# opensensor/thingino-accel

Hardware: AMD Instinct MI355X
Metric: images/sec yolov5s_int8 640x640 batch256 (higher is better)
Workload: dtype int8

## Files before the change

### thingino-accel_amd/csrc/hip/conv_i8_common.hpp

```cpp
#pragma once
#include <hip/hip_runtime.h>
#include <stdint.h>
#include <stdlib.h>
#include <string.h>
#include <type_traits>

#include "../mhip.h"

extern "C" hipStream_t mhip_stream_native(void);
extern "C" int mhip_check(hipError_t e, const char *what);
extern "C" const void *mhip_zero_page(void);

typedef int v4i __attribute__((ext_vector_type(4)));
typedef int v2i __attribute__((ext_vector_type(2)));

#ifdef ANATOMY
struct anat_rec_t {
    unsigned key, wg, hwid, xcc;
    unsigned long long t[4];
};
static __device__ anat_rec_t *g_anat_buf;
static __device__ unsigned g_anat_cap;
#define ANAT_SETTER(NAME)                                                                                                    \
    extern "C" int NAME(void *buf, unsigned cap) {                                                                          \
// ... 82 lines not shown
    const uint32_t b = __builtin_amdgcn_perm((uint32_t)q3, (uint32_t)q2, 0x0c0c0400u);
    return (b << 16) | a;
}
__device__ __forceinline__ void lut4_at0(int q0, int q1, int q2, int q3, int &v0, int &v1, int &v2, int &v3) {
    asm volatile("ds_read_i8 %0, %4 offset:128\n\tds_read_i8 %1, %5 offset:128\n\t"
                 "ds_read_i8 %2, %6 offset:128\n\tds_read_i8 %3, %7 offset:128"
                 : "=&v"(v0), "=&v"(v1), "=&v"(v2), "=&v"(v3)
                 : "v"(q0), "v"(q1), "v"(q2), "v"(q3)
                 : "memory");
}
__device__ __forceinline__ void lds_base_must_be_zero(const void *dynamic_lds) {
    __builtin_amdgcn_s_setprio(3);
    unsigned a = (unsigned)(size_t)(const __attribute__((address_space(3))) void *)dynamic_lds;
    asm volatile("" : "+s"(a));
    if (a != 0u) __builtin_trap();
}
struct add_args_t {
    float s_conv, s_other, inv;
};
__device__ __forceinline__ int add_one(int v, uint32_t xword, int k, const add_args_t &g, int lo8, int hi8) {
    const int x = __builtin_amdgcn_sbfe((int)xword, 8 * k, 8);
    const float y = (float)v * g.s_conv + (float)x * g.s_other;
    const float t = y * g.inv;
    const int r = (int)(t + 0.5f);
    int m;
    asm("v_med3_i32 %0, %1, %2, %3" : "=v"(m) : "v"(r), "v"(lo8), "v"(hi8));
    return m;
}
__device__ __forceinline__ void lut4_fast(int q0, int q1, int q2, int q3, int &v0, int &v1, int &v2, int &v3) {
    asm volatile("ds_read_i8 %0, %4 offset:256\n\tds_read_i8 %1, %5 offset:256\n\t"
                 "ds_read_i8 %2, %6 offset:256\n\tds_read_i8 %3, %7 offset:256"
                 : "=&v"(v0), "=&v"(v1), "=&v"(v2), "=&v"(v3)
                 : "v"(q0), "v"(q1), "v"(q2), "v"(q3)
                 : "memory");
}
template <int NV>
__device__ __forceinline__ void requant_pack_pre(const int (&a)[NV], float cs, uint32_t (&pk)[NV / 4]) {
    const float cs2 = cs * 2.0f;
    const int klo = -256, khi = 255;
    int q[NV], v[NV];
#pragma unroll
    for (int i = 0; i < NV; i++) {
        const int k = (int)((float)a[i] * cs2);
        asm("v_med3_i32 %0, %1, %2, %3" : "=v"(q[i]) : "v"(k), "v"(klo), "v"(khi));
    }
#pragma unroll
    for (int g = 0; g < NV / 4; g++)
        asm volatile("ds_read_i8 %0, %4 offset:768\n\tds_read_i8 %1, %5 offset:768\n\t"
                     "ds_read_i8 %2, %6 offset:768\n\tds_read_i8 %3, %7 offset:768"
                     : "=&v"(v[4 * g]), "=&v"(v[4 * g + 1]), "=&v"(v[4 * g + 2]), "=&v"(v[4 * g + 3])
                     : "v"(q[4 * g]), "v"(q[4 * g + 1]), "v"(q[4 * g + 2]), "v"(q[4 * g + 3])
                     : "memory");
    wait_lds_values<NV>(v);
#pragma unroll
    for (int g = 0; g < NV / 4; g++) pk[g] = pack4(v[4 * g], v[4 * g + 1], v[4 * g + 2], v[4 * g + 3]);
}
__device__ __forceinline__ void requant_pack_two(const int (&a)[16], float cs0, float cs1, uint32_t (&pk)[4]) {
    const float c0 = cs0 * 2.0f, c1 = cs1 * 2.0f;
    const int klo = -256, khi = 255;
    int q[16], v[16];
#pragma unroll
    for (int i = 0; i < 16; i++) {
        const int k = (int)((float)a[i] * (i < 8 ? c0 : c1));
        asm("v_med3_i32 %0, %1, %2, %3" : "=v"(q[i]) : "v"(k), "v"(klo), "v"(khi));
    }
#pragma unroll
    for (int g = 0; g < 2; g++)
        asm volatile("ds_read_i8 %0, %4 offset:768\n\tds_read_i8 %1, %5 offset:768\n\t"
                     "ds_read_i8 %2, %6 offset:768\n\tds_read_i8 %3, %7 offset:768"
                     : "=&v"(v[4 * g]), "=&v"(v[4 * g + 1]), "=&v"(v[4 * g + 2]), "=&v"(v[4 * g + 3])
                     : "v"(q[4 * g]), "v"(q[4 * g + 1]), "v"(q[4 * g + 2]), "v"(q[4 * g + 3])
                     : "memory");
#pragma unroll
    for (int g = 2; g < 4; g++)
        asm volatile("ds_read_i8 %0, %4 offset:1280\n\tds_read_i8 %1, %5 offset:1280\n\t"
                     "ds_read_i8 %2, %6 offset:1280\n\tds_read_i8 %3, %7 offset:1280"
                     : "=&v"(v[4 * g]), "=&v"(v[4 * g + 1]), "=&v"(v[4 * g + 2]), "=&v"(v[4 * g + 3])
                     : "v"(q[4 * g]), "v"(q[4 * g + 1]), "v"(q[4 * g + 2]), "v"(q[4 * g + 3])
                     : "memory");
    wait_lds_values<16>(v);
#pragma unroll
    for (int g = 0; g < 4; g++) pk[g] = pack4(v[4 * g], v[4 * g + 1], v[4 * g + 2], v[4 * g + 3]);
}
template <int NV, bool HAS_LUT, bool SAFE, bool LUT0, bool ADD = false, bool FAST = false>
__device__ __forceinline__ void requant_pack(const int (&a)[NV], float cs, int lo, const uint8_t *lut128, uint32_t (&pk)[NV / 4],
                                             const uint32_t *xw = nullptr, const add_args_t *ga = nullptr) {
    int q[NV];
    const int hi = 127;
    if (FAST && HAS_LUT && LUT0 && SAFE) {
        const float cs2 = cs * 2.0f;
        const int klo = -256, khi = 255;
        int v[NV];
#pragma unroll
        for (int i = 0; i < NV; i++) {
            const int k = (int)((float)a[i] * cs2);
            asm("v_med3_i32 %0, %1, %2, %3" : "=v"(q[i]) : "v"(k), "v"(klo), "v"(khi));
        }
#pragma unroll
        for (int g = 0; g < NV / 4; g++)
            lut4_fast(q[4 * g], q[4 * g + 1], q[4 * g + 2], q[4 * g + 3], v[4 * g], v[4 * g + 1], v[4 * g + 2], v[4 * g + 3]);
        wait_lds_values<NV>(v);
        if (ADD) {
            const int lo8 = -128;
#pragma unroll
            for (int i = 0; i < NV; i++) v[i] = add_one(v[i], xw[i >> 2], i & 3, *ga, lo8, hi);
        }
#pragma unroll
        for (int g = 0; g < NV / 4; g++) pk[g] = pack4(v[4 * g], v[4 * g + 1], v[4 * g + 2], v[4 * g + 3]);
        return;
    }
#pragma unroll
    for (int i = 0; i < NV; i++) q[i] = SAFE ? requant_safe(a[i], cs, lo, hi) : requant<false>(a[i], cs, lo);
    if (HAS_LUT && LUT0) {
        int v[NV];
#pragma unroll
        for (int g = 0; g < NV / 4; g++)
            lut4_at0(q[4 * g], q[4 * g + 1], q[4 * g + 2], q[4 * g + 3], v[4 * g], v[4 * g + 1], v[4 * g + 2], v[4 * g + 3]);
        wait_lds_values<NV>(v);
        if (ADD) {
            const int lo8 = -128;
#pragma unroll
            for (int i = 0; i < NV; i++) v[i] = add_one(v[i], xw[i >> 2], i & 3, *ga, lo8, hi);
        }
#pragma unroll
        for (int g = 0; g < NV / 4; g++) pk[g] = pack4(v[4 * g], v[4 * g + 1], v[4 * g + 2], v[4 * g + 3]);
    } else {
        if (HAS_LUT) {
#pragma unroll
            for (int i = 0; i < NV; i++) q[i] = (int8_t)lut128[q[i]];
        }
        if (ADD) {
            const int lo8 = -128;
#pragma unroll
            for (int i = 0; i < NV; i++) q[i] = add_one(q[i], xw[i >> 2], i & 3, *ga, lo8, hi);
        }
#pragma unroll
        for (int g = 0; g < NV / 4; g++) pk[g] = pack4(q[4 * g], q[4 * g + 1], q[4 * g + 2], q[4 * g + 3]);
    }
}

struct fastdiv_t {
    unsigned m, s1, s2;
};
__device__ __forceinline__ unsigned fdiv(unsigned n, const fastdiv_t d) {
    const unsigned q = __umulhi(d.m, n);
    return (q + ((n - q) >> d.s1)) >> d.s2;
}
static fastdiv_t make_fastdiv(unsigned d) {
    fastdiv_t r;
    unsigned l = 0;
    while ((1ull << l) < d) l++;
    r.m = (unsigned)(((1ull << 32) * ((1ull << l) - d)) / d + 1);
    r.s1 = l < 1 ? l : 1;
    r.s2 = l > 0 ? l - 1 : 0;
    return r;
}

template <int N>
__device__ __forceinline__ void wait_vmcnt() {
    asm volatile("s_waitcnt vmcnt(%0)" ::"n"(N) : "memory");
}

__device__ __forceinline__ void glds16(const void *gsrc, void *lds_wave_base) {
    __builtin_amdgcn_global_load_lds((const __attribute__((address_space(1))) void *)gsrc,
                                     (__attribute__((address_space(3))) void *)lds_wave_base, 16, 0, 0);
}
// ... 187 lines not shown
```

### thingino-accel_amd/csrc/hip/conv_i8_patch.hip

```cpp
#include "conv_i8_common.hpp"
#include <stdio.h>

#ifdef PATCH_STAMPS
__device__ unsigned long long patch_stamp_sums[8];
extern "C" int mhip_patch_stamps(unsigned long long *out, int reset) {
    if (out && hipMemcpyFromSymbol(out, HIP_SYMBOL(patch_stamp_sums), sizeof(patch_stamp_sums)) != hipSuccess) return -1;
    if (reset) {
        unsigned long long z[8] = {0};
        if (hipMemcpyToSymbol(HIP_SYMBOL(patch_stamp_sums), z, sizeof(z)) != hipSuccess) return -1;
    }
    return 0;
}
#define STAMP(t)                                                                          \
    do {                                                                                  \
        __builtin_amdgcn_sched_barrier(0);                                                \
        asm volatile("s_memtime %0\n\ts_waitcnt lgkmcnt(0)" : "=s"(t)::"memory");        \
        __builtin_amdgcn_sched_barrier(0);                                                \
    } while (0)
#else
#define STAMP(t) do { } while (0)
#endif
#define PT_TW 16
#define PT_NIMAX 10

template <int LO, int HI>
__device__ __forceinline__ void wait_vmcnt_tree(int n) {
    if constexpr (LO == HI) {
        wait_vmcnt<LO>();
    } else {
        constexpr int MID = (LO + HI + 1) / 2;
        if (n >= MID) wait_vmcnt_tree<MID, HI>(n);
        else wait_vmcnt_tree<LO, MID - 1>(n);
    }
}
template <int HI>
__device__ __forceinline__ void wait_vmcnt_upto(int n) {
    wait_vmcnt_tree<0, HI>(n > HI ? HI : n);
}
__device__ __forceinline__ void barrier_lds() {
    asm volatile("s_waitcnt lgkmcnt(0)\n\ts_barrier" ::: "memory");
}

template <int TH, int BN, bool HAS_LUT, bool PRE = false, bool POST = false, bool SPLIT = false>
__global__ __launch_bounds__(NTHREADS) void conv_i8_patch(const mhip_conv_i8_t p, const int k64, const int tiles_x,
                                                          const int tiles_y, const unsigned ntiles_all, const int PH,
                                                          const int PW, const int PWP, const int PWH, const int nblk,
                                                          const int8_t *__restrict__ zeros, const fastdiv_t dtx,
                                                          const fastdiv_t dty, const fastdiv_t dpwp, const unsigned out_bytes,
                                                          const int ring, const int xmap, const unsigned in_bytes) {
    ANAT_BEGIN();
    constexpr int WPX = TH / 4;
    constexpr int WOC = BN / 16;
    constexpr int NST = WPX;
    extern __shared__ __attribute__((aligned(16))) int8_t dynlds[];
    uint8_t *slut = (uint8_t *)dynlds;
    lds_base_must_be_zero(dynlds);
    const int nks = k64 / BK;
    constexpr int NPO = 2 * BN;
    static_assert(!SPLIT || (BN == 64 && HAS_LUT && !PRE && !POST), "SPLIT: one 64-channel tile, no other stage");
    constexpr int LB = LUTB + ((PRE || POST) ? 512 : 0) + (SPLIT ? 1024 : 0);
    int *dutab = (int *)(dynlds + LB);
    int8_t *wl = dynlds + LB + ((nks * 16 + 255) & ~255);
    const int patch_bytes = nblk * 1024;
    int8_t *w1l = wl + nks * BN * BK;
    int8_t *pwl = w1l;
    const int *pbl = (const int *)(pwl + NPO * NPO);
    int8_t *swl = w1l;
    const int *sbl = (const int *)(swl + 64 * BK);
    int8_t *patch0 = w1l + (PRE ? p.in_c * BK : 0) + (POST ? NPO * NPO + NPO * 4 : 0) + (SPLIT ? 64 * BK + 64 * 4 : 0);
    int8_t *tpatch = patch0 + ring * patch_bytes;

    const int tid = threadIdx.x, lane = tid & 63;
    const int wv = __builtin_amdgcn_readfirstlane(tid >> 6);
    const int oc0 = blockIdx.y * BN;
    const int C = p.in_c, lgc = 31 - __builtin_clz((unsigned)C), cpp = C >> 4, lgcpp = lgc - 4;
    const int s = p.stride_w;
    const unsigned M = C >= 128 ? 6u : (C >= 64 ? 2u : 0u);

    v4i bias[WOC];
#pragma unroll
    for (int q = 0; q < WOC; q++) bias[q] = p.bias ? *(const v4i *)(p.bias + oc0 + q * 16 + (lane >> 4) * 4) : (v4i){0, 0, 0, 0};
    constexpr int W1MAX = 4;
    v4i pbias[PRE ? W1MAX : 1];
    if (PRE) {
#pragma unroll
        for (int q = 0; q < W1MAX; q++) pbias[q] = q < (C >> 4) ? *(const v4i *)(p.pre_bias + q * 16 + (lane >> 4) * 4) : (v4i){0, 0, 0, 0};
    }
    if (HAS_LUT) {
        if (p.lut2) { if (tid < 128) ((uint32_t *)slut)[tid] = ((const uint32_t *)p.lut2)[tid]; }
        else if (tid < 64) ((uint32_t *)slut)[tid] = ((const uint32_t *)p.lut)[tid];
    }
    if (PRE && tid >= 128) ((uint32_t *)slut)[tid] = ((const uint32_t *)p.pre_lut2)[tid - 128];
    if (POST) {
        if (tid >= 128) ((uint32_t *)slut)[tid] = ((const uint32_t *)p.post_lut2)[tid - 128];
        if (tid < NPO) ((int *)(pwl + NPO * NPO))[tid] = ((const int *)(p.post_w + NPO * NPO))[tid];
    }
    if (SPLIT) {
        if (tid >= 128) {
            ((uint32_t *)slut)[tid] = ((const uint32_t *)p.split_lut2[0])[tid - 128];
            ((uint32_t *)slut)[tid + 128] = ((const uint32_t *)p.split_lut2[1])[tid - 128];
        }
        if (tid < 64) ((int *)(swl + 64 * BK))[tid] = ((const int *)(p.split_w + 64 * BK))[tid];
    }
    const int rowbytes = p.kw * C, kbytes = p.kh * rowbytes;
    for (int i = tid; i < nks * 4; i += NTHREADS) {
        const int kb = i * 16;
        int du = 0;
        if (kb < kbytes) {
            const int ky = kb / rowbytes, rem = kb - ky * rowbytes, kx = rem >> lgc, cc = (rem & (C - 1)) >> 4;
            const int dp = ky * PWP + (s == 2 ? (kx >> 1) + (kx & 1) * PWH : kx);
            du = dp * cpp + cc;
        }
        dutab[i] = du;
    }
    __syncthreads();
    {
        const int schunk = (lane & 3) ^ (((lane >> 4) & 1) << 1);
        for (int i = wv; i < nks * (BN / 16); i += 4) {
            const int ks = i / (BN / 16), g = i - ks * (BN / 16);
            glds16(p.w + (size_t)(oc0 + g * 16 + (lane >> 2)) * k64 + ks * BK + schunk * 16, wl + (ks * BN + g * 16) * BK);
        }
        if (PRE)
            for (int g = wv; g < C / 16; g += 4) glds16(p.pre_w + (size_t)(g * 16 + (lane >> 2)) * BK + schunk * 16, w1l + g * 16 * BK);
        if (POST)
            for (int i = wv; i < NPO * NPO / 1024; i += 4) glds16(p.post_w + i * 1024 + lane * 16, pwl + i * 1024);
        if (SPLIT)
            glds16(p.split_w + wv * 1024 + lane * 16, swl + wv * 1024);
    }
    int uoff[PT_NIMAX], upos[PT_NIMAX];
#pragma unroll
    for (int n = 0; n < PT_NIMAX; n++) {
        uoff[n] = 0;
        upos[n] = -1;
        if (n * 4 + wv < nblk) {
            const unsigned phys = (unsigned)((n * 4 + wv) * 64 + lane);
            const unsigned U = phys ^ ((phys >> 3) & M);
            const unsigned pp = U >> lgcpp, cc = U & (unsigned)(cpp - 1);
            const unsigned py = fdiv(pp, dpwp), col = pp - py * (unsigned)PWP;
            const int px = s == 2 ? ((int)col < PWH ? 2 * (int)col : 2 * ((int)col - PWH) + 1) : (int)col;
            if ((int)py < PH && px < PW) {
                uoff[n] = ((int)py * p.in_w + px) * C + (int)cc * 16;
                upos[n] = ((int)py << 16) | px;
            }
        }
    }
    const int npw = nblk > wv ? (nblk - wv + 3) >> 2 : 0;
    const unsigned xcd = blockIdx.x & 7u;
    const unsigned xstart = xmap ? (unsigned)(((unsigned long long)ntiles_all * xcd) >> 3) : 0u;
    const unsigned xend = xmap ? (unsigned)(((unsigned long long)ntiles_all * (xcd + 1u)) >> 3) : 0u;
    const unsigned ntiles = xmap ? (xend - xstart) * 8u + xcd : ntiles_all;
    auto tile_xy = [&](unsigned t, int &tx, int &ty, unsigned &f) {
        const unsigned j = xmap ? xstart + (t >> 3) : t, q = fdiv(j, dtx);
        tx = (int)(j - q * (unsigned)tiles_x);
        f = fdiv(q, dty);
        ty = (int)(q - f * (unsigned)tiles_y);
    };
    const __amdgpu_buffer_rsrc_t xrs = __builtin_amdgcn_make_buffer_rsrc((void *)p.in, 0, (int)in_bytes, 0x00020000);
    auto issue_patch = [&](unsigned t, int8_t *dst) {
#ifdef PATCH_ABL
        return;
#endif
        int tx, ty;
        unsigned f;
        tile_xy(t, tx, ty, f);
        const int iy0 = ty * TH * s - p.pad_top, ix0 = tx * PT_TW * s - p.pad_left;
        if (in_bytes != 0u && iy0 >= 0 && ix0 >= 0 && iy0 + PH <= p.in_h && ix0 + PW <= p.in_w) {
            const int sbase = (int)(f * (unsigned)p.in_stride) + (iy0 * p.in_w + ix0) * C;
#pragma unroll
            for (int n = 0; n < PT_NIMAX; n++)
                if (n * 4 + wv < nblk) blds16(xrs, uoff[n], sbase, dst + (n * 4 + wv) * 1024);
            return;
        }
        const int8_t *base = p.in + (size_t)f * p.in_stride + ((long)iy0 * p.in_w + ix0) * C;
#pragma unroll
        for (int n = 0; n < PT_NIMAX; n++)
            if (n * 4 + wv < nblk) {
                const int py = upos[n] >> 16, px = upos[n] & 0xffff;
                const bool ok = upos[n] >= 0 && (unsigned)(iy0 + py) < (unsigned)p.in_h && (unsigned)(ix0 + px) < (unsigned)p.in_w;
                glds16(ok ? base + uoff[n] : zeros, dst + (n * 4 + wv) * 1024);
            }
    };

    const __amdgpu_buffer_rsrc_t orsrc = __builtin_amdgcn_make_buffer_rsrc(SPLIT ? p.split_out[0] : (POST ? p.post_out : p.out), 0, (int)out_bytes, 0x00020000);
    const unsigned out_bytes1 = SPLIT ? (unsigned)(p.frames - 1) * (unsigned)p.split_out_stride[1] + (unsigned)(p.out_h * p.out_w) * 32u : 0u;
    const __amdgpu_buffer_rsrc_t orsrc1 = __builtin_amdgcn_make_buffer_rsrc(SPLIT ? p.split_out[1] : p.out, 0, (int)out_bytes1, 0x00020000);
    const bool has_add = !SPLIT && p.add != nullptr;
    constexpr int RROW = WOC == 4 ? 1024 : 512;
    constexpr int NRI = WOC == 4 ? WPX : 2 * WPX;
    int8_t *rstage = patch0 + (ring + (PRE ? 1 : 0)) * patch_bytes + wv * (WPX * RROW);
    const int frow = lane & 15, fchunk = lane >> 4;
    const int chan = (lane >> 4) * (4 * WOC);
    const int NR = has_add || POST ? NRI : 0;
    const int ntail = POST ? (has_add ? NRI : 0) + WPX * (NPO / 64) : (SPLIT ? 2 * WPX : NST);
    const int ppstride = p.post_out_pix_stride ? p.post_out_pix_stride : NPO;
    auto issue_rows = [&](const int8_t *base, size_t fstride, int tx, int ty, unsigned f) {
#pragma unroll
        for (int u = 0; u < WPX; u++) {
            const int oy = ty * TH + wv * WPX + u, ox = tx * PT_TW + frow;
            const int8_t *src = oy < p.out_h && ox < p.out_w ? base + (size_t)f * fstride + ((size_t)(oy * p.out_w + ox) * BN + (size_t)chan) : zeros;
            if (WOC == 4) {
                glds16(src, rstage + u * RROW);
            } else {
                __builtin_amdgcn_global_load_lds((const __attribute__((address_space(1))) void *)src,
                                                 (__attribute__((address_space(3))) void *)(rstage + u * RROW), 4, 0, 0);
                __builtin_amdgcn_global_load_lds((const __attribute__((address_space(1))) void *)(src + 4),
                                                 (__attribute__((address_space(3))) void *)(rstage + u * RROW + 256), 4, 0, 0);
            }
        }
    };
    const int pstride = p.out_pix_stride ? p.out_pix_stride : p.out_c;
    const int lo = p.relu ? 0 : -128;
    const uint8_t *lut128 = slut + 128;
    int ubase[WPX];
#pragma unroll
    for (int u = 0; u < WPX; u++) ubase[u] = ((wv * WPX + u) * s * PWP + frow) * cpp;

    const unsigned G = gridDim.x;
    const int D = ring - 1;
    unsigned t = blockIdx.x;
    int yg0 = 0, yg1 = 0, yg2 = 0;
    {
        int issued = 0;
        for (int d = 0; d < D; d++)
            if (t + (unsigned)d * G < ntiles) {
                issue_patch(t + (unsigned)d * G, patch0 + d * patch_bytes);
                issued++;
            }
        yg0 = issued > 1 ? (issued - 1) * npw : 0;
        yg1 = issued > 2 ? (issued - 2) * npw : 0;
        yg2 = 0;
    }
#ifdef PATCH_STAMPS
    unsigned long long st0 = 0, st1 = 0, st2 = 0, st3 = 0, st4 = 0, sum_wait = 0, sum_issue = 0, sum_k = 0, sum_epi = 0, sum_tiles = 0;
#endif
    int cur = 0;
    int pn_last = 0;
    bool first = true;
    ANAT_NOW(1);
    for (; t < ntiles; t += G) {
        STAMP(st0);
        int tx, ty;
        unsigned f;
        tile_xy(t, tx, ty, f);
        int voffs[WPX];
        uint32_t xw[WPX][WOC];
#pragma unroll
        for (int u = 0; u < WPX; u++) {
            const int oy = ty * TH + wv * WPX + u, ox = tx * PT_TW + frow;
            const unsigned off = f * (unsigned)p.out_stride + (unsigned)(oy * p.out_w + ox) * (unsigned)pstride +
                                 (unsigned)(p.out_ch_off + oc0 + chan);
            const bool ok = oy < p.out_h && ox < p.out_w && oc0 + chan < p.out_c;
            voffs[u] = ok ? (int)off : -1;
#pragma unroll
            for (int q = 0; q < WOC; q++) xw[u][q] = 0;
        }
        if (POST) {
#pragma unroll
            for (int u = 0; u < WPX; u++) {
                const int oy = ty * TH + wv * WPX + u, ox = tx * PT_TW + frow;
                const unsigned off = f * (unsigned)p.post_out_stride + (unsigned)(oy * p.out_w + ox) * (unsigned)ppstride +
                                     (unsigned)(p.post_out_ch_off + (lane >> 4) * (NPO / 4));
                voffs[u] = oy < p.out_h && ox < p.out_w ? (int)off : -1;
            }
            if (has_add) issue_rows(p.add, p.out_stride, tx, ty, f);
            else issue_rows(p.post_in, p.post_in_stride, tx, ty, f);
        } else if (SPLIT) {
#pragma unroll
            for (int u = 0; u < WPX; u++) {
                const int oy = ty * TH + wv * WPX + u, ox = tx * PT_TW + frow;
                voffs[u] = oy < p.out_h && ox < p.out_w ? (oy * p.out_w + ox) * 32 + (lane >> 4) * 8 : -1;
            }
        } else if (has_add) {
#pragma unroll
            for (int u = 0; u < WPX; u++) {
                const int8_t *src = voffs[u] >= 0 ? p.add + (unsigned)voffs[u] : zeros;
                if (WOC == 4) {
// ... 116 lines not shown
            du_n = dutab[clampk(ks + 2) * 4 + fchunk];
            __builtin_amdgcn_sched_barrier(0);
            mfma_step(xb, wb);
            __builtin_amdgcn_sched_barrier(0);
            load_frags(clampk(ks + 2), du_n, xb, wb);
            du_n = dutab[clampk(ks + 3) * 4 + fchunk];
            __builtin_amdgcn_sched_barrier(0);
            mfma_step(xa, wa);
            __builtin_amdgcn_sched_barrier(0);
        }
        if (ks < nks) mfma_step(xb, wb);
        STAMP(st3);
        if (D > 0) cur = cur + 1 == ring ? 0 : cur + 1;
        if (has_add) {
            if (D > 0) wait_vmcnt_upto<15>(pn_last);
#pragma unroll
            for (int u = 0; u < WPX; u++) {
                if (WOC == 4) {
                    const v4i r = *(const v4i *)(rstage + u * RROW + lane * 16);
                    xw[u][0] = (uint32_t)r[0]; xw[u][1] = (uint32_t)r[1]; xw[u][WOC > 2 ? 2 : 0] = (uint32_t)r[2]; xw[u][WOC > 3 ? 3 : 0] = (uint32_t)r[3];
                } else {
                    xw[u][0] = *(const uint32_t *)(rstage + u * RROW + lane * 4);
                    xw[u][WOC > 1 ? 1 : 0] = *(const uint32_t *)(rstage + u * RROW + 256 + lane * 4);
                }
            }
        }
        uint32_t pku[POST || SPLIT ? WPX : 1][WOC];
        if (POST && has_add) {
#pragma unroll
            for (int u = 0; u < WPX; u++) {
                if constexpr (WOC == 4) asm volatile("s_waitcnt lgkmcnt(0)" : "+v"(xw[u][0]), "+v"(xw[u][1]), "+v"(xw[u][2]), "+v"(xw[u][3])::"memory");
                else asm volatile("s_waitcnt lgkmcnt(0)" : "+v"(xw[u][0]), "+v"(xw[u][1])::"memory");
            }
            issue_rows(p.post_in, p.post_in_stride, tx, ty, f);
        }
#pragma unroll
        for (int u = 0; u < WPX; u++) {
            uint32_t pk[WOC];
            int a[WOC * 4];
#pragma unroll
            for (int q = 0; q < WOC; q++)
#pragma unroll
                for (int r = 0; r < 4; r++) a[q * 4 + r] = acc[q][u][r];
            const bool fast = HAS_LUT && p.lut2 != nullptr;
            if (has_add) {
                const add_args_t ga = {p.add_s_conv, p.add_s_other, p.add_inv};
                if (fast) requant_pack<WOC * 4, HAS_LUT, true, true, true, true>(a, p.cs, lo, lut128, pk, xw[u], &ga);
                else requant_pack<WOC * 4, HAS_LUT, true, true, true>(a, p.cs, lo, lut128, pk, xw[u], &ga);
            } else {
                if (fast) requant_pack<WOC * 4, HAS_LUT, true, true, false, true>(a, p.cs, lo, lut128, pk);
                else requant_pack<WOC * 4, HAS_LUT, true, true>(a, p.cs, lo, lut128, pk);
            }
            if (POST) {
#pragma unroll
                for (int q = 0; q < WOC; q++) pku[POST ? u : 0][q] = pk[q];
                continue;
            }
            if (SPLIT) {
#pragma unroll
                for (int q = 0; q < WOC; q++) pku[SPLIT ? u : 0][q] = pk[q];
                continue;
            }
            const int voff = voffs[u];
            if (WOC == 4)
                __builtin_amdgcn_raw_buffer_store_b128((v4i){(int)pk[0], (int)pk[1], (int)pk[2], (int)pk[3]}, orsrc, voff, 0, 0);
            else if (WOC == 2)
                __builtin_amdgcn_raw_buffer_store_b64((v2i){(int)pk[0], (int)pk[WOC > 1 ? 1 : 0]}, orsrc, voff, 0, 0);
        }
        if (SPLIT) {
            v4i sw4[4], sb4[4];
#pragma unroll
            for (int r = 0; r < 4; r++) {
                sw4[r] = *(const v4i *)(swl + lds_off(r * 16 + frow, fchunk));
                sb4[r] = *(const v4i *)(sbl + r * 16 + fchunk * 4);
            }
            v4i sc[WPX][4];
#pragma unroll
            for (int u = 0; u < WPX; u++) {
                const v4i b0 = {(int)pku[SPLIT ? u : 0][0], (int)pku[SPLIT ? u : 0][1], (int)pku[SPLIT ? u : 0][WOC > 2 ? 2 : 0], (int)pku[SPLIT ? u : 0][WOC > 3 ? 3 : 0]};
#pragma unroll
                for (int r = 0; r < 4; r++) sc[u][r] = __builtin_amdgcn_mfma_i32_16x16x64_i8(sw4[r], b0, sb4[r], 0, 0, 0);
            }
            const unsigned fo0 = f * (unsigned)p.split_out_stride[0], fo1 = f * (unsigned)p.split_out_stride[1];
#pragma unroll
            for (int u = 0; u < WPX; u++) {
                int a2[16];
#pragma unroll
                for (int r = 0; r < 4; r++)
#pragma unroll
                    for (int e = 0; e < 4; e++) a2[r * 4 + e] = sc[u][r][e];
                uint32_t pk4[4];
                requant_pack_two(a2, p.split_cs[0], p.split_cs[1], pk4);
                const int voff0 = voffs[u] >= 0 ? voffs[u] + (int)fo0 : -1, voff1 = voffs[u] >= 0 ? voffs[u] + (int)fo1 : -1;
                __builtin_amdgcn_raw_buffer_store_b64((v2i){(int)pk4[0], (int)pk4[1]}, orsrc, voff0, 0, 0);
                __builtin_amdgcn_raw_buffer_store_b64((v2i){(int)pk4[2], (int)pk4[3]}, orsrc1, voff1, 0, 0);
            }
        }
        if (POST) {
            if (has_add) wait_vmcnt<0>();
            else if (D > 0) wait_vmcnt_upto<15>(pn_last);
#pragma unroll
            for (int u = 0; u < WPX; u++) {
                v4i b0, b1 = {0, 0, 0, 0};
                if (WOC == 4) {
                    b0 = (v4i){(int)pku[POST ? u : 0][0], (int)pku[POST ? u : 0][1], (int)pku[POST ? u : 0][WOC > 2 ? 2 : 0], (int)pku[POST ? u : 0][WOC > 3 ? 3 : 0]};
                    b1 = *(const v4i *)(rstage + u * RROW + lane * 16);
                } else {
                    b0 = (v4i){(int)pku[POST ? u : 0][0], (int)pku[POST ? u : 0][WOC > 1 ? 1 : 0], *(const int *)(rstage + u * RROW + lane * 4),
                               *(const int *)(rstage + u * RROW + 256 + lane * 4)};
                }
#pragma unroll
                for (int h = 0; h < NPO / 64; h++) {
                    int a[16];
#pragma unroll
                    for (int s4 = 0; s4 < 4; s4++) {
                        const int row = (h * 4 + s4) * 16;
                        v4i c = *(const v4i *)(pbl + row + fchunk * 4);
                        c = __builtin_amdgcn_mfma_i32_16x16x64_i8(*(const v4i *)(pwl + lds_off(row + frow, fchunk)), b0, c, 0, 0, 0);
                        if (WOC == 4) c = __builtin_amdgcn_mfma_i32_16x16x64_i8(*(const v4i *)(pwl + NPO * BK + lds_off(row + frow, fchunk)), b1, c, 0, 0, 0);
#pragma unroll
                        for (int e = 0; e < 4; e++) a[s4 * 4 + e] = c[e];
                    }
                    uint32_t pk4[4];
                    requant_pack_pre<16>(a, p.post_cs, pk4);
                    const int voff = voffs[u] >= 0 ? voffs[u] + h * 16 : -1;
                    __builtin_amdgcn_raw_buffer_store_b128((v4i){(int)pk4[0], (int)pk4[1], (int)pk4[2], (int)pk4[3]}, orsrc, voff, 0, 0);
                }
            }
        }
#ifdef PATCH_STAMPS
        STAMP(st4);
        if (D == 0) st1 = st2;
        sum_wait += st1 - st0; sum_issue += st2 - st1; sum_k += st3 - st2; sum_epi += st4 - st3; sum_tiles += 1;
#endif
    }
    ANAT_NOW(2);
    ANAT_END(p);
#ifdef PATCH_STAMPS
    if (lane == 0) {
        atomicAdd(&patch_stamp_sums[0], sum_wait); atomicAdd(&patch_stamp_sums[1], sum_issue); atomicAdd(&patch_stamp_sums[2], sum_k);
        atomicAdd(&patch_stamp_sums[3], sum_epi); atomicAdd(&patch_stamp_sums[4], sum_tiles);
    }
#endif
}

ANAT_SETTER(mhip_anatomy_set_patch)
struct patch_geom_t {
    int bn, tiles_x, tiles_y, PH, PW, PWP, PWH, nblk, nks, ring;
    size_t lds;
};
static inline const tune_t &tune() { return conv_i8_tune_state(); }
static size_t patch_lds_budget(int bn) {
    const int kb = tune().patch_lds_kb;
    if (kb >= 16 && kb <= 160 && kb != 80) return (size_t)kb * 1024;
    return (size_t)(bn == 32 ? 53 : 80) * 1024;
}
static bool patch_geom(const mhip_conv_i8_t *p, int th, patch_geom_t *g) {
    const bool direct = conv_i8_direct_rows(p);
    const int C = p->in_c, s = p->stride_w;
    static const bool no_c16 = getenv("MARS_HIP_PATCH_NO_C16") != nullptr;
    if (!direct || !p->safe || (C != 16 && C != 32 && C != 64 && C != 128) || (C == 16 && (no_c16 || p->pre_w)) || (s != 1 && s != 2) || p->stride_h != s ||
        p->kh > 7 || p->kw > 7 || p->kh * p->kw < 2 || p->row_pad != p->kw * C || persist_out_bytes(p) > 0x7fffffffL)
        return false;
    const int k64 = (p->kh * p->row_pad + BK - 1) / BK * BK;
    g->nks = k64 / BK;
    g->bn = p->oc_pad % 64 == 0 ? 64 : 32;
    g->tiles_x = (p->out_w + PT_TW - 1) / PT_TW;
    g->tiles_y = (p->out_h + th - 1) / th;
    if ((double)p->out_h * p->out_w < (C == 128 ? 0.80 : 0.85) * (double)g->tiles_x * PT_TW * g->tiles_y * th) return false;
    g->PH = (th - 1) * s + p->kh;
    g->PW = (PT_TW - 1) * s + p->kw;
    g->PWH = s == 2 ? (g->PW + 1) / 2 : 0;
    g->PWP = s == 2 ? 2 * g->PWH : g->PW;
    const long units = (long)g->PH * g->PWP * (C / 16);
    g->nblk = (int)((units + 63) / 64);
    if (g->nblk > 4 * PT_NIMAX) return false;
    const bool pre = p->pre_w != nullptr;
    if (pre && (s != 1 || (C != 32 && C != 64) || !p->pre_bias || !p->pre_lut2 || !p->lut2)) return false;
    const bool post = p->post_w != nullptr;
    if (post) {
        const long ppstride = p->post_out_pix_stride ? p->post_out_pix_stride : 2 * g->bn;
        if (pre || s != 1 || p->out_c != g->bn || p->oc_pad != g->bn || p->out_pix_stride || p->out_ch_off || !p->lut2 || !p->post_lut2 || !p->post_in ||
            !p->post_out || ((p->post_out_pix_stride | p->post_out_ch_off) & 15) || p->post_out_pix_stride < 0 || p->post_out_ch_off < 0 ||
            ppstride < p->post_out_ch_off + 2 * g->bn ||
            (long)(p->frames - 1) * (long)p->post_out_stride + (long)p->out_h * p->out_w * ppstride > 0x7fffffffL)
            return false;
    }
    const bool split = p->split_w != nullptr;
    if (split) {
        if (pre || post || p->add || g->bn != 64 || p->out_c != 64 || p->oc_pad != 64 || p->out_pix_stride || p->out_ch_off || !p->lut2 || !p->split_lut2[0] ||
            !p->split_lut2[1] || !p->split_out[0] || !p->split_out[1])
            return false;
        for (int i = 0; i < 2; i++)
            if ((long)(p->frames - 1) * (long)p->split_out_stride[i] + (long)p->out_h * p->out_w * 32 > 0x7fffffffL) return false;
    }
    const size_t pb = (size_t)g->nblk * 1024;
    const size_t radd = p->add || post ? (size_t)4 * (th / 4) * (g->bn == 64 ? 1024 : 512) : 0;
    const size_t fixed = LUTB + (pre ? 512 + (size_t)C * BK + pb : 0) + (post ? 512 + (size_t)4 * g->bn * g->bn + (size_t)8 * g->bn : 0) +
                         (split ? 1024 + (size_t)64 * BK + 64 * 4 : 0) +
                         (((size_t)g->nks * 16 + 255) & ~(size_t)255) + (size_t)g->nks * g->bn * BK + radd;
    const size_t budget = patch_lds_budget(g->bn);
    if (fixed + pb > budget) return false;
    const int fit = (int)((budget - fixed) / pb);
    const int cap = tune().patch_ring > 0 ? (tune().patch_ring > 4 ? 4 : tune().patch_ring) : 2;
    int ring = fit < cap ? fit : cap;
    g->ring = ring;
    g->lds = fixed + (size_t)ring * pb;
    if ((long)g->tiles_x * g->tiles_y * p->frames > 0x7fffffffL) return false;
    return true;
}

static inline long post_out_bytes(const mhip_conv_i8_t *p) {
    const long ppstride = p->post_out_pix_stride ? p->post_out_pix_stride : 2 * p->out_c;
    return (long)(p->frames - 1) * (long)p->post_out_stride + (long)p->out_h * p->out_w * ppstride;
}
static inline long split_out_bytes(const mhip_conv_i8_t *p, int side) {
    return (long)(p->frames - 1) * (long)p->split_out_stride[side] + (long)p->out_h * p->out_w * 32;
}
template <int TH, int BN, bool HAS_LUT, bool PRE = false, bool POST = false, bool SPLIT = false>
static int launch_patch_t(const mhip_conv_i8_t *p, int k64, const patch_geom_t &g) {
    auto kern = conv_i8_patch<TH, BN, HAS_LUT, PRE, POST, SPLIT>;
    static int cus = 0;
    static size_t slots_lds[8];
    static int slots_n[8], nslots = 0;
    if (!cus) {
        int dev = 0;
        hipDeviceProp_t prop;
        if (hipFuncSetAttribute((const void *)kern, hipFuncAttributeMaxDynamicSharedMemorySize, 160 * 1024) != hipSuccess ||
            hipGetDevice(&dev) != hipSuccess || hipGetDeviceProperties(&prop, dev) != hipSuccess)
            return mhip_check(hipErrorUnknown, "conv_i8_patch occupancy query");
        cus = prop.multiProcessorCount;
    }
    int slots = 0;
    for (int i = 0; i < nslots; i++)
        if (slots_lds[i] == g.lds) slots = slots_n[i];
    if (!slots) {
        int occ = 0;
        if (hipOccupancyMaxActiveBlocksPerMultiprocessor(&occ, kern, NTHREADS, g.lds) != hipSuccess)
            return mhip_check(hipErrorUnknown, "conv_i8_patch occupancy query");
        slots = (occ > 0 ? occ : 1) * cus;
        if (nslots < 8) { slots_lds[nslots] = g.lds; slots_n[nslots++] = slots; }
    }
    const unsigned ntiles = (unsigned)((long)g.tiles_x * g.tiles_y * p->frames);
    const unsigned noc = (unsigned)(p->oc_pad / BN);
    unsigned gx = (unsigned)(tune().persist_slots > 0 ? tune().persist_slots : slots) / noc;
    if (gx < 1) gx = 1;
    if (gx > ntiles) gx = ntiles;
    const int xmap = gx >= 8 && ntiles < 0x0fffffffu;
    if (xmap) gx &= ~7u;
    {
        static const char *dbg = getenv("MARS_HIP_PATCH_DEBUG");
        static size_t last_lds = 0;
        static int last_ring = 0;
        if (dbg && (last_lds != g.lds || last_ring != g.ring)) {
            fprintf(stderr, "Mars: conv_i8_patch<%d,%d> ring %d, patch %d KB, LDS %zu B, %d workgroups per CU, grid %u x %u\n", TH, BN, g.ring,
                    g.nblk, g.lds, slots / cus, gx, noc);
            last_lds = g.lds;
            last_ring = g.ring;
        }
    }
    hipLaunchKernelGGL(kern, dim3(gx, noc), dim3(NTHREADS), g.lds, mhip_stream_native(), *p, k64,
                       g.tiles_x, g.tiles_y, ntiles, g.PH, g.PW, g.PWP, g.PWH, g.nblk, (const int8_t *)mhip_zero_page(),
                       make_fastdiv((unsigned)g.tiles_x), make_fastdiv((unsigned)g.tiles_y), make_fastdiv((unsigned)g.PWP),
                       (unsigned)(SPLIT ? split_out_bytes(p, 0) : (POST ? post_out_bytes(p) : persist_out_bytes(p))), g.ring, xmap,
                       in_extent_bytes(p) <= 0x7fffffffL ? (unsigned)in_extent_bytes(p) : 0u);
    return mhip_check(hipGetLastError(), "conv_i8_patch launch");
}

bool conv_i8_patch_ok(const mhip_conv_i8_t *p, int th, int *ring) {
    patch_geom_t g;
    if (!patch_geom(p, th, &g)) return false;
    if (ring) *ring = g.ring;
    return true;
}

int conv_i8_launch_patch(const mhip_conv_i8_t *p, int k64, int th) {
    patch_geom_t g;
    if (!patch_geom(p, th, &g)) return -1;
#define PATCH(T, B)                                                                       \
    (p->post_w ? launch_patch_t<T, B, true, false, true>(p, k64, g)                       \
     : p->pre_w ? launch_patch_t<T, B, true, true>(p, k64, g)                             \
                : (p->lut ? launch_patch_t<T, B, true>(p, k64, g) : launch_patch_t<T, B, false>(p, k64, g)))
    if (p->split_w) {
        if (th == 16) return launch_patch_t<16, 64, true, false, false, true>(p, k64, g);
        if (th == 8) return launch_patch_t<8, 64, true, false, false, true>(p, k64, g);
        return launch_patch_t<4, 64, true, false, false, true>(p, k64, g);
    }
    if (th == 16) return g.bn == 64 ? PATCH(16, 64) : PATCH(16, 32);
    if (th == 8) return g.bn == 64 ? PATCH(8, 64) : PATCH(8, 32);
    return g.bn == 64 ? PATCH(4, 64) : PATCH(4, 32);
#undef PATCH
}

int conv_i8_pre_tile_rows(const mhip_conv_i8_t *p) {
    patch_geom_t g;
    for (int th : {16, 8, 4})
        if (patch_geom(p, th, &g) && (th == 4 || g.ring >= 2)) return th;
    return 0;
}
extern "C" int mhip_conv_i8_pre_ok(const mhip_conv_i8_t *p) {
    if (!p || !p->pre_w || p->nseg > 1 || p->out_nchw) return 0;
    return conv_i8_pre_tile_rows(p) != 0;
}

int conv_i8_post_tile_rows(const mhip_conv_i8_t *p) {
    patch_geom_t g;
    for (int th : {16, 8, 4})
        if (patch_geom(p, th, &g)) return th;
    return 0;
}
extern "C" int mhip_conv_i8_post_ok(const mhip_conv_i8_t *p) {
    if (!p || !p->post_w || p->pre_w || p->nseg > 1 || p->out_nchw) return 0;
    return conv_i8_post_tile_rows(p) != 0;
}
extern "C" int mhip_conv_i8_post_k(int c, int k) {
    if (c == 64) return k;
    return k < 32 ? (k >> 3) * 16 + (k & 7) : ((k - 32) >> 3) * 16 + 8 + (k & 7);
}
extern "C" int mhip_conv_i8_post_row(int c, int oc) {
    const int per = c / 2, g = oc / per, rem = oc - g * per;
    return (rem >> 2) * 16 + g * 4 + (rem & 3);
}
extern "C" size_t mhip_conv_i8_post_pack(int c, const int8_t *packed, const int32_t *bias, int8_t *out) {
    if (c != 32 && c != 64) return 0;
    const int n = 2 * c;
    const size_t bytes = (size_t)n * n + (size_t)n * 4;
    if (!packed || !out) return bytes;
    memset(out, 0, bytes);
    for (int oc = 0; oc < n; oc++) {
        const int R = mhip_conv_i8_post_row(c, oc), src = mhip_conv_i8_oc_row(oc, n);
        for (int k = 0; k < n; k++) {
            const int pos = mhip_conv_i8_post_k(c, k), ks = pos >> 6, chunk = (pos & 63) >> 4;
            out[(size_t)(ks * n + R) * BK + (((chunk ^ ((R >> 1) & 2))) << 4) + (pos & 15)] = packed[(size_t)src * n + k];
        }
        ((int32_t *)(out + (size_t)n * n))[R] = bias ? bias[src] : 0;
    }
    return bytes;
}

int conv_i8_split_tile_rows(const mhip_conv_i8_t *p) {
    patch_geom_t g;
    for (int th : {16, 8, 4})
        if (patch_geom(p, th, &g)) return th;
    return 0;
}
extern "C" int mhip_conv_i8_split_ok(const mhip_conv_i8_t *p) {
    if (!p || !p->split_w || p->pre_w || p->post_w || p->add || p->nseg > 1 || p->out_nchw) return 0;
    return conv_i8_split_tile_rows(p) != 0;
}
extern "C" int mhip_conv_i8_split_row(int side, int oc) {
    const int g = oc >> 3, rem = oc & 7;
    return side * 32 + (rem >> 2) * 16 + g * 4 + (rem & 3);
}
extern "C" size_t mhip_conv_i8_split_pack(const int8_t *packed0, const int32_t *bias0, const int8_t *packed1, const int32_t *bias1, int8_t *out) {
    const size_t bytes = (size_t)64 * BK + (size_t)64 * 4;
    if (!packed0 || !packed1 || !out) return bytes;
    memset(out, 0, bytes);
    for (int side = 0; side < 2; side++) {
        const int8_t *packed = side ? packed1 : packed0;
        const int32_t *bias = side ? bias1 : bias0;
        for (int oc = 0; oc < 32; oc++) {
            const int R = mhip_conv_i8_split_row(side, oc), src = mhip_conv_i8_oc_row(oc, 32);
            for (int k = 0; k < 64; k++) out[(size_t)R * BK + ((((k >> 4) ^ ((R >> 1) & 2))) << 4) + (k & 15)] = packed[(size_t)src * 64 + k];
            ((int32_t *)(out + (size_t)64 * BK))[R] = bias ? bias[src] : 0;
        }
    }
    return bytes;
}
```

### thingino-accel_amd/csrc/host/mars_internal.h

```cpp
#ifndef MARS_INTERNAL_H
#define MARS_INTERNAL_H

#include <stddef.h>
#include <stdint.h>

#include "../mhip.h"
#include "mars_hip.h"
#include "mars_runtime.h"

enum {
    OP_CONV_I8 = 0,
    OP_CONV_F32,
    OP_RELU_BYTES,
    OP_LUT_I8,
    OP_BINARY_I8,
    OP_SIGMOID_F32,
    OP_BINARY_F32,
    OP_RELU_F32,
    OP_BN,
    OP_MAXPOOL,
    OP_CONCAT_SLICE,
    OP_UPSAMPLE,
    OP_UPSAMPLE_Q, OP_MAXPOOL_Q,
    OP_CONCAT_Q,
    OP_CONV_F32_VHEAD,
    OP_FAIL,
};

#define NO_OFF ((size_t)-1)
#define MARS_MAX_IO 4
#define MARS_MAX_MODEL_TUNE 16

typedef struct {
    size_t bytes;
    size_t extent;
    size_t stride;
    uint8_t *dev;
    int is_weight;
    int needed;
    int io_in, io_out;
    uint8_t *host;
    uint8_t *dense_dev;
    int pix_c, pix_stride;
    int rec_c, rec_hw;
    int nhwc_c, nhwc_hw;
    size_t zero_from;
    int partial;
    int nhwc_pitch;
    int tail_read;
} mtensor_t;

typedef struct {
    int kind, layer, err;
    int t_in[4], n_in, t_out;
    int in_h, in_w, in_c, out_h, out_w, out_c, kh, kw, sh, sw, pt, pl;
    int nchw, relu, is_mul, is_f32, leaky, safe;
    size_t in_byte_off, out_byte_off;
    int k_limit;
    int vc_n, vc_t[3], vc_run, vc_shift;
    int rows_only;
    int out_nchw;
    int silu_f32;
    int f32_exact;
    int variant;
    int add_t; float add_s_conv, add_s_other, add_inv;
    int nseg, seg_t[4], seg_c[4], seg_up;
    int chain_n, chain_out[3];
    int pair_next;
    int row_pad, oc_pad, c_pad;
    int ch_off, scale_h, scale_w, bn_n;
    int out_pix_stride, out_ch_off;
    int store_c;
    float cs, f0, f1, f2;
    size_t n;
    size_t w_off, b_off, lut_off, s_off;
    int pre;
    size_t pre_w_off, pre_b_off, pre_lut2_off;
    float pre_cs;
    int post_next;
    size_t post_w_off;
    int split_next;
    size_t split_w_off;
    size_t w2_off;
    int w2_rows;
    int w2_planes;
    size_t w3_off;
    int w3_stem;
    int in_rec, out_rec;
    size_t lut2_off;
    size_t w_blob_off[2];
    double macs, bytes;
    int prof_kind;
    float last_ms;
    void *ev0, *ev1;
    int prof_rec;
    void *ev_start;
} mars_op_t;

typedef struct {
    int fusion;
    unsigned no_fuse_lut : 1, no_nhwc_internal : 1, no_vconcat_q : 1, no_pair_f32 : 1, no_rec : 1, no_zero_tail : 1, no_vconcat_f32 : 1,
        no_rowpad : 1, no_post : 1, no_split : 1;
    size_t rec_limit;
    size_t vconcat_limit;
    size_t bottleneck_limit;
} plan_switches_t;

typedef struct mars_model_ext {
    mars_model_t pub;
    plan_switches_t sw;
    int batch, profiling, deferred;
    int plan_err;
    int no_vconcat;
    int no_download;
    int no_bottleneck;
    int no_post;
    int no_split;
    int rec_frames;
    int rec_skipped;
    size_t rec_max_frames;
    mtensor_t *mt;
    mars_op_t *ops;
    int n_ops, cap_ops;
    uint8_t *arena_host;
    size_t arena_size, arena_cap;
    uint8_t *arena_dev;
    size_t blob_mirror_bytes;
    uint8_t *act_dev;
    size_t act_bytes;
    uint8_t *scratch_dev;
    size_t scratch_per_frame;
    int scratch_t, scratch_cpad, scratch_f0, scratch_n;
    void *det_dev;
    int *det_counts_dev;
    float *det_lut_dev;
    int det_cap;
    float det_lut_scale[4];
    int det_lut_n;
    int det_lut_mono[4];
    float *heads_lut_dev;
    float heads_lut_scale[4];
    int heads_lut_n;
    float *dfl_lut_dev;
    float dfl_lut_scale[4][2];
    int dfl_lut_n;
    void *ev_graph_done, *ev_tail_done;
    int tail_pending;
    int frame0, run_frames;
    void *ev_fork, *ev_join[3];
    void *ev_chunk[2][8];
    void *graph_exec;
    unsigned graph_gen;
    int ran_plain;
    void *pipe;
    struct { char key[28]; int value, saved; } tune[MARS_MAX_MODEL_TUNE];
    int n_tune, tune_depth;
    int plan_f32_mode;
    unsigned char *layer_noop;
    void *roi_dev;
    int roi_cap_slots, roi_cap_frames;
    int roi_slots;
    struct mars_model_ext *roi_from;
    void *cls_dev;
    size_t cls_bytes, cls_sums_off, cls_top_off;
    int cls_frames, cls_c, cls_top_k;
    void *ev_label_done;
    int label_pending;
    void *label_dev;
    int label_cap, label_frames;
    void *match_dev;
    size_t match_bytes, match_top_off, match_row_off;
    int match_frames, match_top_k;
    void *ident_dev;
    int ident_cap, ident_frames;
    void *track_dev;
    int track_cap, track_frames;
    void *seg_dev;
    size_t seg_bytes, seg_rec_off, seg_word_off;
    int seg_frames, seg_max, seg_ph, seg_pw;
    void *ev_seg[2];
    void *pose_dev;
    size_t pose_bytes, pose_rec_off, pose_kpt_off;
    int pose_frames, pose_max, pose_k;
    float pose_lut_scale[4];
    int pose_lut_n;
    void *ev_pose[2];
    void *obb_dev;
    size_t obb_bytes, obb_cnt_off, obb_out_off;
    int obb_frames;
    float obb_lut_scale[4];
    int obb_lut_n;
    void *ev_obb[2];
    int det_mapped;
    void *tile_roi_dev;
    int tile_roi_cap;
    void *tile_dev;
    int tile_cap, tile_cams;
    void *ev_tile[2];
    struct mars_model_ext *live_next;
} mars_model_ext_t;


#define MARS_INTERNAL __attribute__((visibility("hidden")))
#define ALIGN_UP(x, a) (((x) + (size_t)(a) - 1) & ~((size_t)(a) - 1))
#define NO_TENSOR 0xFFFFFFFFu
#define MAX_DIM_PRODUCT ((size_t)1 << 40)
#define ARENA_MAX ((size_t)1 << 40)
#define MAX_CHANNELS 65536
MARS_INTERNAL int mars_verbose(void);
#define VLOG(...) do { if (mars_verbose()) fprintf(stderr, "Mars: " __VA_ARGS__); } while (0)
MARS_INTERNAL void drop_graph(mars_model_ext_t *m);
MARS_INTERNAL mars_model_ext_t *mars_live_models(void);
MARS_INTERNAL void plan_switches_read(plan_switches_t *sw, int at_load);
MARS_INTERNAL mars_error_t build_plan(mars_model_ext_t *m);
MARS_INTERNAL mars_error_t upload_params(mars_model_ext_t *m);
MARS_INTERNAL mars_error_t alloc_batch(mars_model_ext_t *m, int n);
MARS_INTERNAL size_t elem_size(uint32_t dtype);
MARS_INTERNAL size_t shape_numel(const mars_tensor_t *d);
MARS_INTERNAL size_t reference_buffer_size(const mars_model_ext_t *m);
MARS_INTERNAL size_t arena_reserve(mars_model_ext_t *m, size_t bytes);
MARS_INTERNAL void blob_read(const mars_model_ext_t *m, size_t off, size_t n, void *dst);
MARS_INTERNAL int op_reads(const mars_op_t *o, int t);
MARS_INTERNAL int op_writes(const mars_op_t *o, int t);
MARS_INTERNAL size_t planned_stride(const mtensor_t *t);
MARS_INTERNAL void conv_i8_geometry(const mars_op_t *op, int frames, mhip_conv_i8_t *p);
MARS_INTERNAL int conv_i8_pre_fits(const mars_op_t *op, int frames, size_t in_stride, size_t out_stride);
MARS_INTERNAL int conv_i8_post_fits(const mars_model_ext_t *m, const mars_op_t *a, const mars_op_t *b, int frames);
MARS_INTERNAL int conv_i8_split_fits(const mars_model_ext_t *m, const mars_op_t *a, const mars_op_t *b, const mars_op_t *c, int frames);
MARS_INTERNAL void plan_layer(mars_model_ext_t *m, int li);
MARS_INTERNAL void fold_silu(mars_model_ext_t *m, int f32);
MARS_INTERNAL void fuse_lut(mars_model_ext_t *m);
MARS_INTERNAL void nhwc_internal(mars_model_ext_t *m);
MARS_INTERNAL void fold_add(mars_model_ext_t *m, int f32);
MARS_INTERNAL void virtual_concat(mars_model_ext_t *m);
MARS_INTERNAL void elide_concat(mars_model_ext_t *m);
MARS_INTERNAL void trim_concat(mars_model_ext_t *m);
MARS_INTERNAL void fuse_pool_chains(mars_model_ext_t *m);
MARS_INTERNAL void pair_convs(mars_model_ext_t *m);
MARS_INTERNAL void fuse_bottleneck(mars_model_ext_t *m);
MARS_INTERNAL void fuse_post(mars_model_ext_t *m);
MARS_INTERNAL void fuse_split(mars_model_ext_t *m);
MARS_INTERNAL void pad_output_rows(mars_model_ext_t *m);
MARS_INTERNAL void virtual_concat_q(mars_model_ext_t *m);
MARS_INTERNAL void f32_policy(mars_model_ext_t *m);
MARS_INTERNAL void zero_tail_f32(mars_model_ext_t *m);
MARS_INTERNAL void pair_convs_f32(mars_model_ext_t *m);
MARS_INTERNAL void rec_pairs(mars_model_ext_t *m);
MARS_INTERNAL void virtual_concat_f32(mars_model_ext_t *m);
MARS_INTERNAL void plan_check(mars_model_ext_t *m);
MARS_INTERNAL void conv_i8_params(const mars_model_ext_t *m, const mars_op_t *op, mhip_conv_i8_t *p);
MARS_INTERNAL int mars_preproc_prepare(int w, int h, int tw, int th);
MARS_INTERNAL int mars_preproc_prepare_nv12(int w, int h, int tw, int th, int frames);

MARS_INTERNAL void mars_roi_release(mars_model_ext_t *m);

MARS_INTERNAL void mars_cls_release(mars_model_ext_t *m);

MARS_INTERNAL void mars_match_release(mars_model_ext_t *m);

MARS_INTERNAL void mars_track_release(mars_model_ext_t *m);

MARS_INTERNAL void mars_seg_release(mars_model_ext_t *m);

MARS_INTERNAL void mars_pose_release(mars_model_ext_t *m);

MARS_INTERNAL void mars_obb_release(mars_model_ext_t *m);

MARS_INTERNAL void mars_tile_release(mars_model_ext_t *m);

MARS_INTERNAL int mars_tensor_chw(const mars_tensor_t *d, int *c, int *h, int *w);
MARS_INTERNAL int mars_locate_i8(const mars_model_ext_t *m, int T, int ch, int hh, int ww, int any_writer, int *buf, int *off, int *pix_step, int *ch_step);
MARS_INTERNAL mars_error_t mars_own_det_buffers(mars_model_ext_t *m);
MARS_INTERNAL mars_error_t mars_tail_on_aux(mars_model_ext_t *m, int (*launch)(struct mars_model_ext *, const void *, void *, int *), const void *cfg);

mars_error_t mars_detect_prepare(mars_model_ext_t *m, const int *output_indices, int n_outputs);
int mars_detect_launch(mars_model_ext_t *m, const int *output_indices, int n_outputs, float nms_thresh, void *dets_dev,
                       int *counts_dev);

typedef struct {
    int n, ti[4], stride[4], nc[4], h[4], w[4], pix_step[4], ch_step[4];
    float anchors[4][3][2];
    float conf, nms;
    int map, px, py;
    float rx, ry;
    int internal;
} mars_heads_cfg_t;
MARS_INTERNAL int mars_find_heads(const mars_model_ext_t *m, int *tensor_ids, int *strides, int *num_classes, int cap);
MARS_INTERNAL mars_error_t mars_heads_resolve(mars_model_ext_t *m, const mars_yolo_heads_t *h, mars_heads_cfg_t *c);
MARS_INTERNAL mars_error_t mars_heads_prepare(mars_model_ext_t *m, const mars_heads_cfg_t *c);
MARS_INTERNAL int mars_heads_launch(mars_model_ext_t *m, const mars_heads_cfg_t *c, void *dets_dev, int *counts_dev);

typedef struct {
    int n, reg_max, stride[4], nc[4], h[4], w[4];
    int box_t[4], cls_t[4], box_buf[4], cls_buf[4], box_off[4], cls_off[4];
    int box_pix_step[4], box_ch_step[4], cls_pix_step[4], cls_ch_step[4];
    float box_scale[4], cls_scale[4];
    float conf, nms;
    int map, px, py;
    float rx, ry;
    int internal;
    int *cand_pred, *kept_pred;
    void *premap;
} mars_dfl_cfg_t;
MARS_INTERNAL int mars_find_dfl_heads(const mars_model_ext_t *m, int *box_ids, int *cls_ids, int *strides, int *num_classes, int *reg_max, int cap);
MARS_INTERNAL mars_error_t mars_dfl_resolve(mars_model_ext_t *m, const mars_yolo_dfl_heads_t *h, mars_dfl_cfg_t *c);
MARS_INTERNAL mars_error_t mars_dfl_prepare(mars_model_ext_t *m, const mars_dfl_cfg_t *c);
MARS_INTERNAL int mars_dfl_launch(mars_model_ext_t *m, const mars_dfl_cfg_t *c, void *dets_dev, int *counts_dev);

int32_t mars_trunc_x86(float x);
void mars_pack_conv_i8(const int8_t *w, size_t avail, int nchw, int out_c, int in_c, int kh, int kw,
                       int c_pad, int row_pad, int oc_pad, int8_t *dst);

#endif
```

### thingino-accel_amd/csrc/host/mars_model.c

```c
#include <math.h>
#include <stdio.h>
#include <stdlib.h>
#include <string.h>
#include <sys/types.h>
#include <time.h>

#include "mars_internal.h"
#include "nna.h"


int mars_verbose(void) {
    static int v = -1;
    if (v < 0) v = getenv("MARS_VERBOSE") ? 1 : 0;
    return v;
}

void plan_switches_read(plan_switches_t *sw, int at_load) {
    const char *e;
    if (at_load) sw->fusion = (e = getenv("MARS_HIP_FUSION")) ? atoi(e) : 1;
    sw->no_fuse_lut = getenv("MARS_HIP_NO_FUSE_LUT") != NULL;
    sw->no_nhwc_internal = getenv("MARS_HIP_NO_NHWC_INTERNAL") != NULL;
    sw->no_vconcat_q = getenv("MARS_HIP_NO_VCONCAT_Q") != NULL;
    sw->no_pair_f32 = getenv("MARS_HIP_NO_PAIR_F32") != NULL;
    sw->no_rec = getenv("MARS_HIP_NO_REC") != NULL;
    sw->no_zero_tail = getenv("MARS_HIP_NO_ZERO_TAIL") != NULL;
    sw->no_vconcat_f32 = getenv("MARS_HIP_NO_VCONCAT_F32") != NULL;
    sw->no_rowpad = getenv("MARS_HIP_NO_ROWPAD") != NULL;
    sw->no_post = getenv("MARS_HIP_NO_POST") != NULL;
    sw->no_split = getenv("MARS_HIP_NO_SPLIT") != NULL;
    sw->rec_limit = (e = getenv("MARS_HIP_REC_LIMIT")) ? (size_t)strtoull(e, NULL, 0) : (size_t)0xfffffff0u;
    sw->vconcat_limit = (e = getenv("MARS_HIP_VCONCAT_LIMIT")) ? (size_t)strtoull(e, NULL, 0) : (size_t)0x7fffffffu;
    sw->bottleneck_limit = (e = getenv("MARS_HIP_BOTTLENECK_LIMIT")) ? (size_t)strtoull(e, NULL, 0) : 0;
}

void drop_graph(mars_model_ext_t *m) {
    if (m->graph_exec) {
        mhip_sync();
        mhip_graph_destroy(m->graph_exec);
    }
    m->graph_exec = NULL;
    m->ran_plain = 0;
}

static const char *const k_err[] = {
    "OK", "Invalid magic number", "Version mismatch", "Memory allocation failed",
    "Invalid file format", "NNA initialization failed", "Layer execution failed",
    "Invalid tensor", "Invalid layer",
};

const char *mars_get_error_string(mars_error_t err) {
    int i = -(int)err;
    if (i >= 0 && i < (int)(sizeof(k_err) / sizeof(k_err[0]))) return k_err[i];
    return "Unknown error";
}

static void free_device_state(mars_model_ext_t *m) {
    drop_graph(m);
    if (m->act_dev) mhip_free(m->act_dev);
    if (m->scratch_dev) mhip_free(m->scratch_dev);
    m->act_dev = m->scratch_dev = NULL;
    for (uint32_t i = 0; m->mt && i < m->pub.header.num_tensors; i++) {
        if (m->mt[i].host) mhip_host_free(m->mt[i].host);
        m->mt[i].host = NULL;
        if (m->mt[i].dense_dev) mhip_free(m->mt[i].dense_dev);
        m->mt[i].dense_dev = NULL;
        if (!m->mt[i].is_weight) m->mt[i].dev = NULL;
    }
    if (m->det_dev) mhip_free(m->det_dev);
    if (m->det_counts_dev) mhip_free(m->det_counts_dev);
    m->det_dev = NULL;
    m->det_counts_dev = NULL;
    m->det_cap = 0;
    m->tail_pending = 0;
    mars_roi_release(m);
    mars_cls_release(m);
    mars_track_release(m);
    mars_seg_release(m);
    mars_pose_release(m);
    mars_obb_release(m);
    mars_tile_release(m);
}

static void free_ops(mars_model_ext_t *m) {
    drop_graph(m);
    for (int i = 0; i < m->n_ops; i++) {
        if (m->ops[i].ev0) mhip_event_destroy(m->ops[i].ev0);
        if (m->ops[i].ev1) mhip_event_destroy(m->ops[i].ev1);
    }
    free(m->ops);
    m->ops = NULL;
    m->n_ops = m->cap_ops = 0;
}

static mars_model_ext_t *g_live_models = NULL;
mars_model_ext_t *mars_live_models(void) { return g_live_models; }

void mars_free(mars_model_t *model) {
    if (!model) return;
    mars_model_ext_t *m = (mars_model_ext_t *)model;
    for (mars_model_ext_t **pp = &g_live_models; *pp; pp = &(*pp)->live_next)
        if (*pp == m) { *pp = m->live_next; break; }
    for (mars_model_ext_t *x = g_live_models; x; x = x->live_next)
        if (x->roi_from == m) x->roi_from = NULL;
    if (m->pipe) mars_hip_pipe_close(model);
    if (mhip_ready()) mhip_sync();
    free_device_state(m);
    free_ops(m);
    if (m->arena_dev) mhip_free(m->arena_dev);
    if (m->det_lut_dev) mhip_free(m->det_lut_dev);
    if (m->heads_lut_dev) mhip_free(m->heads_lut_dev);
    if (m->dfl_lut_dev) mhip_free(m->dfl_lut_dev);
    if (m->ev_graph_done) mhip_event_destroy(m->ev_graph_done);
    if (m->ev_tail_done) mhip_event_destroy(m->ev_tail_done);
    if (m->ev_label_done) mhip_event_destroy(m->ev_label_done);
    if (m->ev_fork) mhip_event_destroy(m->ev_fork);
    for (int k = 0; k < 3; k++)
        if (m->ev_join[k]) mhip_event_destroy(m->ev_join[k]);
    for (int k = 0; k < 2; k++)
        for (int c = 0; c < 8; c++)
            if (m->ev_chunk[k][c]) mhip_event_destroy(m->ev_chunk[k][c]);
    free(m->arena_host);
    free(m->layer_noop);
    free(m->mt);
    free(m->pub.weights);
    free(m->pub.layers);
    free(m->pub.tensors);
    free(m);
}

mars_error_t build_plan(mars_model_ext_t *m) {
    const uint32_t nt = m->pub.header.num_tensors, nl = m->pub.header.num_layers;
    plan_switches_read(&m->sw, 0);
    free_ops(m);
    m->arena_size = 0;
    if (m->arena_host) memset(m->arena_host, 0, m->arena_cap);
    m->scratch_per_frame = 0;
    m->plan_err = MARS_OK;
    m->plan_f32_mode = mhip_conv_f32_mode(-1);
    m->blob_mirror_bytes = m->pub.weights_size;
    for (uint32_t i = 0; i < nt; i++) {
        m->mt[i].extent = m->mt[i].bytes;
        m->mt[i].pix_c = m->mt[i].pix_stride = 0;
        m->mt[i].needed = (m->mt[i].io_in || m->mt[i].io_out) ? 1 : 0;
    }
    for (uint32_t i = 0; i < nl && m->plan_err == MARS_OK; i++) {
        const int n0 = m->n_ops;
        plan_layer(m, (int)i);
        m->layer_noop[i] = m->n_ops == n0;
    }
    if (m->plan_err != MARS_OK) return (mars_error_t)m->plan_err;
    if (m->sw.fusion >= 1) {
        fold_silu(m, 0);
        fuse_lut(m);
        fold_silu(m, 1);
        nhwc_internal(m);
        fold_add(m, 0);
        fold_add(m, 1);
        if (!m->no_vconcat) virtual_concat(m);
        elide_concat(m);
        trim_concat(m);
        fuse_pool_chains(m);
        pair_convs(m);
        if (m->sw.fusion >= 2 && !m->no_bottleneck) fuse_bottleneck(m);
        fuse_post(m);
        fuse_split(m);
        pad_output_rows(m);
        virtual_concat_q(m);
    } else {
        nhwc_internal(m);
    }
    f32_policy(m);
    zero_tail_f32(m);
    if (m->sw.fusion >= 1) pair_convs_f32(m);
    rec_pairs(m);
    virtual_concat_f32(m);
    if (m->plan_err == MARS_OK) plan_check(m);
    return (mars_error_t)m->plan_err;
}

mars_error_t upload_params(mars_model_ext_t *m) {
    size_t mirror_off = arena_reserve(m, m->blob_mirror_bytes + 64);
    if (mirror_off == NO_OFF) return MARS_ERR_ALLOC_FAILED;
    if (!m->deferred) blob_read(m, 0, m->blob_mirror_bytes, m->arena_host + mirror_off);
    if (m->arena_dev) mhip_free(m->arena_dev);
    m->arena_dev = (uint8_t *)mhip_malloc(m->arena_size);
    if (!m->arena_dev) return MARS_ERR_ALLOC_FAILED;
    if (mhip_h2d_async(m->arena_dev, m->arena_host, m->arena_size) || mhip_sync()) return MARS_ERR_NNA_INIT_FAILED;
    for (uint32_t i = 0; i < m->pub.header.num_tensors; i++) {
        if (!m->mt[i].is_weight) continue;
        m->mt[i].dev = m->arena_dev + mirror_off + (size_t)m->pub.tensors[i].desc.data_offset;
        m->mt[i].stride = 0;
        m->pub.tensors[i].paddr = m->mt[i].dev;
    }
    m->pub.ddr_paddr = m->arena_dev;
    m->pub.ddr_size = m->arena_size;
    return MARS_OK;
}

mars_error_t alloc_batch(mars_model_ext_t *m, int n) {
    const uint32_t nt = m->pub.header.num_tensors;
    if (m->pipe) mars_hip_pipe_close(&m->pub);
    if (mhip_sync()) return MARS_ERR_LAYER_FAILED;
    plan_switches_read(&m->sw, 0);
    const size_t vlim = m->sw.vconcat_limit, blim = m->sw.bottleneck_limit;
    const int rec_replan = (size_t)n > m->rec_max_frames || (m->rec_skipped && n < m->rec_frames);
    m->rec_frames = n;
    if (m->no_vconcat || m->no_bottleneck || m->no_post || m->no_split || rec_replan) {
        m->no_vconcat = m->no_bottleneck = m->no_post = m->no_split = 0;
        mars_error_t e = build_plan(m);
        if (e == MARS_OK) e = upload_params(m);
        if (e != MARS_OK) return e;
    }
    if (!m->no_vconcat)
        for (int i = 0; i < m->n_ops; i++) {
            const mars_op_t *op = &m->ops[i];
            if (op->kind != OP_CONV_I8 || op->nseg < 2 || op->t_out < 0) continue;
            if (planned_stride(&m->mt[op->t_out]) * (size_t)n > vlim) {
                m->no_vconcat = 1;
                mars_error_t e = build_plan(m);
                if (e == MARS_OK) e = upload_params(m);
                if (e != MARS_OK) return e;
                break;
            }
        }
    if (m->sw.fusion >= 2 && !m->no_bottleneck)
        for (int i = 0; i < m->n_ops; i++) {
            const mars_op_t *op = &m->ops[i];
            if (op->kind != OP_CONV_I8 || !op->pre || op->t_out < 0) continue;
            const size_t in_stride = op->t_in[0] >= 0 ? planned_stride(&m->mt[op->t_in[0]]) : 0;
            if (!conv_i8_pre_fits(op, n, in_stride, planned_stride(&m->mt[op->t_out])) || (blim && (size_t)n > blim)) {
                m->no_bottleneck = 1;
                mars_error_t e = build_plan(m);
                if (e == MARS_OK) e = upload_params(m);
                if (e != MARS_OK) return e;
                break;
            }
        }
    if (!m->no_post)
        for (int i = 0; i + 1 < m->n_ops; i++) {
            const mars_op_t *op = &m->ops[i];
            if (op->kind != OP_CONV_I8 || !op->post_next) continue;
            if (!conv_i8_post_fits(m, op, op + 1, n)) {
                m->no_post = 1;
                mars_error_t e = build_plan(m);
                if (e == MARS_OK) e = upload_params(m);
                if (e != MARS_OK) return e;
                break;
            }
        }
    if (!m->no_split)
        for (int i = 0; i + 2 < m->n_ops; i++) {
            const mars_op_t *op = &m->ops[i];
            if (op->kind != OP_CONV_I8 || !op->split_next) continue;
            if (!conv_i8_split_fits(m, op, op + 1, op + 2, n)) {
                m->no_split = 1;
                mars_error_t e = build_plan(m);
                if (e == MARS_OK) e = upload_params(m);
                if (e != MARS_OK) return e;
                break;
            }
        }
    free_device_state(m);
    size_t per_frame = 0;
    for (uint32_t i = 0; i < nt; i++) {
        mtensor_t *t = &m->mt[i];
        if (t->is_weight || !t->needed) continue;
        t->stride = planned_stride(t);
        per_frame += t->stride;
    }
    m->act_bytes = per_frame * (size_t)n;
    m->act_dev = (uint8_t *)mhip_malloc(m->act_bytes + 512);
    if (!m->act_dev) return MARS_ERR_ALLOC_FAILED;
    if (mhip_memset_async(m->act_dev, 0, m->act_bytes + 256)) return MARS_ERR_ALLOC_FAILED;
    size_t off = 256;
    for (uint32_t i = 0; i < nt; i++) {
        mtensor_t *t = &m->mt[i];
        mars_runtime_tensor_t *rt = &m->pub.tensors[i];
        if (t->is_weight) continue;
        rt->vaddr = NULL; rt->paddr = NULL; rt->alloc_size = 0;
        if (!t->needed) continue;
        t->dev = m->act_dev + off;
        off += t->stride * (size_t)n;
        rt->paddr = t->dev;
        rt->alloc_size = t->stride * (size_t)n;
        if (t->io_in || t->io_out) {
            const size_t hb = t->bytes * (size_t)n, ref = reference_buffer_size(m);
            size_t cap = hb > ref ? hb : ref;
            if (ref > ((size_t)8 << 20)) cap = hb;
            t->host = (uint8_t *)mhip_host_alloc(cap ? cap : 64);
            if (!t->host) return MARS_ERR_ALLOC_FAILED;
            memset(t->host, 0, cap);
            rt->vaddr = t->host;
            rt->alloc_size = n == 1 && cap >= ref ? ref : hb;
        }
        if (t->pix_stride) {
            t->dense_dev = (uint8_t *)mhip_malloc(t->bytes * (size_t)n);
            if (!t->dense_dev) return MARS_ERR_ALLOC_FAILED;
        }
    }
    if (m->scratch_per_frame) {
        m->scratch_dev = (uint8_t *)mhip_malloc(ALIGN_UP(m->scratch_per_frame, 256) * (size_t)n + 256);
        if (!m->scratch_dev) return MARS_ERR_ALLOC_FAILED;
    }
    m->batch = n;
    m->frame0 = 0;
    m->run_frames = n;
    return mhip_sync() ? MARS_ERR_ALLOC_FAILED : MARS_OK;
}

static mars_error_t load_host(const void *data, size_t size, unsigned flags, mars_model_ext_t **out_m) {
    if (!data || !out_m || size < sizeof(mars_header_t)) return MARS_ERR_INVALID_FILE;
    const uint8_t *p = (const uint8_t *)data;
    mars_header_t h;
    memcpy(&h, p, sizeof(h));
    if (h.magic != MARS_MAGIC) {
        VLOG("Invalid magic 0x%08x (expected 0x%08x)\n", h.magic, MARS_MAGIC);
        return MARS_ERR_INVALID_MAGIC;
    }
    if (h.version_major != MARS_VERSION_MAJOR) return MARS_ERR_VERSION_MISMATCH;
    if (h.num_tensors > 65536 || h.num_layers > 65536 || h.num_inputs > 4 || h.num_outputs > 4) return MARS_ERR_INVALID_FILE;
    const size_t tables = sizeof(h) + (size_t)h.num_tensors * sizeof(mars_tensor_t) + (size_t)h.num_layers * sizeof(mars_layer_t);
    if (tables > size) return MARS_ERR_INVALID_FILE;
    const int deferred = (flags & MARS_HIP_LOAD_DEFER_WEIGHTS) != 0;
    if (!deferred && h.weights_size > 0 && (h.weights_offset > size || h.weights_size > size - h.weights_offset))
        return MARS_ERR_INVALID_FILE;
    if (h.weights_size > ((uint64_t)1 << 36)) return MARS_ERR_INVALID_FILE;
// ... 6 lines not shown
    m->pub.tensors = (mars_runtime_tensor_t *)calloc(h.num_tensors ? h.num_tensors : 1, sizeof(mars_runtime_tensor_t));
    m->pub.layers = (mars_runtime_layer_t *)calloc(h.num_layers ? h.num_layers : 1, sizeof(mars_runtime_layer_t));
    m->mt = (mtensor_t *)calloc(h.num_tensors ? h.num_tensors : 1, sizeof(mtensor_t));
    m->layer_noop = (unsigned char *)calloc(h.num_layers ? h.num_layers : 1, 1);
    if (!m->pub.tensors || !m->pub.layers || !m->mt || !m->layer_noop) { mars_free(&m->pub); return MARS_ERR_ALLOC_FAILED; }
    const uint8_t *q = p + sizeof(h);
    for (uint32_t i = 0; i < h.num_tensors; i++, q += sizeof(mars_tensor_t)) memcpy(&m->pub.tensors[i].desc, q, sizeof(mars_tensor_t));
    for (uint32_t i = 0; i < h.num_layers; i++, q += sizeof(mars_layer_t)) memcpy(&m->pub.layers[i].desc, q, sizeof(mars_layer_t));

    m->pub.weights_size = (size_t)h.weights_size;
    if (h.weights_size) {
        m->pub.weights = calloc(1, (size_t)h.weights_size);
        if (!m->pub.weights) { mars_free(&m->pub); return MARS_ERR_ALLOC_FAILED; }
        if (!deferred) memcpy(m->pub.weights, p + h.weights_offset, (size_t)h.weights_size);
    }
    m->pub.ddr_base = m->pub.weights;
    for (uint32_t i = 0; i < h.num_tensors; i++) {
        mars_runtime_tensor_t *rt = &m->pub.tensors[i];
        if (rt->desc.ndims > MARS_MAX_DIMS) { mars_free(&m->pub); return MARS_ERR_INVALID_FILE; }
        m->mt[i].bytes = shape_numel(&rt->desc) * elem_size(rt->desc.dtype);
        if (rt->desc.data_size > 0) {
            if (rt->desc.data_offset > h.weights_size) { mars_free(&m->pub); return MARS_ERR_INVALID_FILE; }
            m->mt[i].is_weight = 1;
            rt->vaddr = (uint8_t *)m->pub.weights + rt->desc.data_offset;
            rt->alloc_size = (size_t)rt->desc.data_size;
        }
    }
    for (uint32_t i = 0; i < h.num_inputs; i++) {
        uint32_t id = h.input_tensor_ids[i];
        if (id < h.num_tensors && !m->mt[id].is_weight) m->mt[id].io_in = (int)i + 1;
    }
    for (uint32_t i = 0; i < h.num_outputs; i++) {
        uint32_t id = h.output_tensor_ids[i];
        if (id < h.num_tensors && !m->mt[id].is_weight) m->mt[id].io_out = (int)i + 1;
    }

    mars_error_t err = build_plan(m);
    if (err != MARS_OK) { mars_free(&m->pub); return err; }
    VLOG("%u layers -> %d launches, parameter arena %zu bytes\n", h.num_layers, m->n_ops, m->arena_size);
    *out_m = m;
    return MARS_OK;
}

mars_error_t mars_hip_load_memory_ex(const void *data, size_t size, unsigned flags, mars_model_t **out_model) {
    if (!out_model) return MARS_ERR_INVALID_FILE;
    mars_model_ext_t *m = NULL;
    mars_error_t err = load_host(data, size, flags, &m);
    if (err != MARS_OK) return err;
    if (!nna_is_ready() || !mhip_ready()) {
        fprintf(stderr, "Mars: no initialised MI355X device (call nna_init first); refusing to load\n");
        mars_free(&m->pub);
        return MARS_ERR_NNA_INIT_FAILED;
    }
    err = upload_params(m);
    if (err == MARS_OK) err = alloc_batch(m, 1);
    if (err != MARS_OK) { mars_free(&m->pub); return err; }
    m->live_next = g_live_models;
    g_live_models = m;
    *out_model = &m->pub;
    return MARS_OK;
}

static int describe_op_full(const mars_op_t *o, char *line, size_t cap, int k) {
#define ADD(...) k += snprintf(line + k, cap - (size_t)k, __VA_ARGS__)
    ADD(" | err %d in %dx%dx%d out %dx%dx%d k %dx%d s %dx%d p %d,%d", o->err, o->in_h, o->in_w, o->in_c, o->out_h, o->out_w, o->out_c, o->kh, o->kw, o->sh, o->sw, o->pt, o->pl);
    ADD(" nchw %d out_nchw %d relu %d is_mul %d is_f32 %d leaky %d safe %d silu %d f32_exact %d variant %d", o->nchw, o->out_nchw, o->relu, o->is_mul, o->is_f32, o->leaky,
        o->safe, o->silu_f32, o->f32_exact, o->variant);
    ADD(" row_pad %d oc_pad %d c_pad %d store_c %d ch_off %d out_ch_off %d out_pix_stride %d in_byte_off %zu out_byte_off %zu scale %dx%d bn_n %d n %zu", o->row_pad,
        o->oc_pad, o->c_pad, o->store_c, o->ch_off, o->out_ch_off, o->out_pix_stride, o->in_byte_off, o->out_byte_off, o->scale_h, o->scale_w, o->bn_n, o->n);
    ADD(" k_limit %d rows_only %d pair_next %d in_rec %d out_rec %d vc %d,%d,%d:", o->k_limit, o->rows_only, o->pair_next, o->in_rec, o->out_rec, o->vc_n, o->vc_run, o->vc_shift);
    for (int q = 0; q < o->vc_n && q < 3; q++) ADD(" %d", o->vc_t[q]);
    ADD(" add %d %a %a %a seg %d up %d:", o->add_t, (double)o->add_s_conv, (double)o->add_s_other, (double)o->add_inv, o->nseg, o->seg_up);
    for (int q = 0; q < o->nseg && q < 4; q++) ADD(" %d/%d", o->seg_t[q], o->seg_c[q]);
    ADD(" chain %d:", o->chain_n);
    for (int q = 0; q < o->chain_n && q < 3; q++) ADD(" %d", o->chain_out[q]);
    ADD(" cs %a f %a %a %a", (double)o->cs, (double)o->f0, (double)o->f1, (double)o->f2);
    ADD(" w_off %zd b_off %zd lut_off %zd lut2_off %zd s_off %zd w2_off %zd rows %d planes %d w3_off %zd stem %d blob %zd %zd", (ssize_t)o->w_off, (ssize_t)o->b_off,
        (ssize_t)o->lut_off, (ssize_t)o->lut2_off, (ssize_t)o->s_off, (ssize_t)o->w2_off, o->w2_rows, o->w2_planes, (ssize_t)o->w3_off, o->w3_stem, (ssize_t)o->w_blob_off[0],
        (ssize_t)o->w_blob_off[1]);
    ADD(" post_next %d", o->post_next);
    if (o->post_next) ADD(" %zd", (ssize_t)o->post_w_off);
    ADD(" split_next %d", o->split_next);
    if (o->split_next) ADD(" %zd", (ssize_t)o->split_w_off);
    ADD(" pre %d", o->pre);
    if (o->pre) ADD(" %zd %zd %zd %a", (ssize_t)o->pre_w_off, (ssize_t)o->pre_b_off, (ssize_t)o->pre_lut2_off, (double)o->pre_cs);
    ADD(" macs %a bytes %a prof_kind %d", o->macs, o->bytes, o->prof_kind);
#undef ADD
    return k;
}

size_t mars_hip_describe_plan(const void *data, size_t size, unsigned flags, char *out, size_t cap) {
    static const char *const kinds[] = {"conv_i8", "conv_f32", "relu_bytes", "lut_i8", "binary_i8", "sigmoid_f32", "binary_f32", "relu_f32", "bn",
                                        "maxpool", "concat_slice", "upsample", "upsample_q", "maxpool_q", "concat_q", "conv_f32_vhead", "fail"};
    mars_model_ext_t *m = NULL;
    const int full = (flags & MARS_HIP_DESCRIBE_FULL) != 0;
    if (load_host(data, size, flags & ~MARS_HIP_DESCRIBE_FULL, &m) != MARS_OK) return 0;
    size_t n = 0;
    char line[4096];
#define EMIT() do { const size_t l = strlen(line); if (out && n < cap) memcpy(out + n, line, n + l <= cap ? l : cap - n); n += l; } while (0)
    for (int i = 0; i < m->n_ops; i++) {
        const mars_op_t *o = &m->ops[i];
        int k = snprintf(line, sizeof line, "op %d layer %d %s in", i, o->layer, o->kind >= 0 && o->kind <= OP_FAIL ? kinds[o->kind] : "?");
        for (int q = 0; q < o->n_in && q < 4; q++) k += snprintf(line + k, sizeof line - (size_t)k, " %d", o->t_in[q]);
        k += snprintf(line + k, sizeof line - (size_t)k, " out %d", o->t_out);
#define FLAG(cond, ...) if (cond) k += snprintf(line + k, sizeof line - (size_t)k, __VA_ARGS__)
        FLAG(o->kind == OP_CONV_I8 || o->kind == OP_CONV_F32 || o->kind == OP_CONV_F32_VHEAD, " k%dx%d s%d c%d->%d", o->kh, o->kw, o->sw, o->in_c, o->out_c);
        FLAG(o->nchw, " relayout"); FLAG(o->out_nchw, " planar_store"); FLAG(o->lut_off != NO_OFF, " lut"); FLAG(o->add_t, " add=%d", o->add_t - 1);
        FLAG(o->nseg, " seg=%d", o->nseg); FLAG(o->pair_next, " pair_next"); FLAG(o->post_next, " post_next"); FLAG(o->split_next, " split_next"); FLAG(o->pre, " pre"); FLAG(o->silu_f32, " silu");
        FLAG(o->k_limit, " k_limit=%d", o->k_limit); FLAG(o->in_rec, " in_rec=%d", o->in_rec); FLAG(o->out_rec, " out_rec");
        FLAG(o->vc_shift, " view=-%d", o->vc_shift); FLAG(o->vc_n, " vcat=%dx%d", o->vc_n, o->vc_run);
        FLAG(o->rows_only, " rows_only=%d", o->rows_only); FLAG(o->out_byte_off, " out_off=%zu", o->out_byte_off); FLAG(o->chain_n, " chain=%d", o->chain_n);
        FLAG(o->out_pix_stride, " pix_stride=%d", o->out_pix_stride); FLAG(o->kind == OP_FAIL, " err=%d", o->err);
#undef FLAG
        if (full) k = describe_op_full(o, line, sizeof line, k);
        snprintf(line + k, sizeof line - (size_t)k, "\n");
        EMIT();
    }
    for (uint32_t t = 0; t < m->pub.header.num_tensors; t++) {
        const mtensor_t *mt = &m->mt[t];
        const int listed = mt->nhwc_c || mt->partial || mt->zero_from || mt->rec_c || mt->pix_stride;
        if (!listed && !(full && mt->needed)) continue;
        int k = listed ? snprintf(line, sizeof line, "tensor %u nhwc_c %d pitch %d partial %d zero_from %zu rec_c %d pix_stride %d", t, mt->nhwc_c, mt->nhwc_pitch,
                                  mt->partial, mt->zero_from, mt->rec_c, mt->pix_stride)
                       : snprintf(line, sizeof line, "+tensor %u", t);
        if (full)
            k += snprintf(line + k, sizeof line - (size_t)k, " | bytes %zu extent %zu needed %d tail_read %d weight %d io %d,%d pix_c %d rec_hw %d nhwc_hw %d", mt->bytes,
                          mt->extent, mt->needed, mt->tail_read, mt->is_weight, mt->io_in, mt->io_out, mt->pix_c, mt->rec_hw, mt->nhwc_hw);
        snprintf(line + k, sizeof line - (size_t)k, "\n");
        EMIT();
    }
    if (full) {
        const plan_switches_t *w = &m->sw;
        snprintf(line, sizeof line, "+plan n_ops %d arena_size %zu scratch_per_frame %zu blob_mirror_bytes %zu rec_max_frames %zu rec_skipped %d f32_mode %d | fusion %d"
                 " no_fuse_lut %d no_nhwc_internal %d no_vconcat_q %d no_pair_f32 %d no_rec %d no_zero_tail %d no_vconcat_f32 %d no_rowpad %d no_post %d no_split %d rec_limit %zu"
                 " vconcat_limit %zu bottleneck_limit %zu\n", m->n_ops, m->arena_size, m->scratch_per_frame, m->blob_mirror_bytes, m->rec_max_frames, m->rec_skipped,
                 m->plan_f32_mode, w->fusion, w->no_fuse_lut, w->no_nhwc_internal, w->no_vconcat_q, w->no_pair_f32, w->no_rec, w->no_zero_tail, w->no_vconcat_f32,
                 w->no_rowpad, w->no_post, w->no_split, w->rec_limit, w->vconcat_limit, w->bottleneck_limit);
        EMIT();
    }
#undef EMIT
    if (out && cap) out[n < cap ? n : cap - 1] = 0;
    mars_free(&m->pub);
    return n;
}

int mars_yolo_find_heads(const void *data, size_t size, int *tensor_ids, int *strides, int *num_classes, int cap) {
    mars_model_ext_t *m = NULL;
    if (load_host(data, size, 0, &m) != MARS_OK) return -1;
    const int n = mars_find_heads(m, tensor_ids, strides, num_classes, cap);
    mars_free(&m->pub);
    return n;
}

int mars_yolo_find_dfl_heads(const void *data, size_t size, int *box_ids, int *cls_ids, int *strides, int *num_classes, int *reg_max, int cap) {
    mars_model_ext_t *m = NULL;
    if (load_host(data, size, 0, &m) != MARS_OK) return -1;
    const int n = mars_find_dfl_heads(m, box_ids, cls_ids, strides, num_classes, reg_max, cap);
    mars_free(&m->pub);
    return n;
}

mars_error_t mars_load_memory(const void *data, size_t size, mars_model_t **model) {
    return mars_hip_load_memory_ex(data, size, 0, model);
}

mars_error_t mars_load_file(const char *path, mars_model_t **model) {
    if (!path || !model) return MARS_ERR_INVALID_FILE;
    FILE *fp = fopen(path, "rb");
    if (!fp) {
        fprintf(stderr, "Mars: Cannot open %s\n", path);
        return MARS_ERR_INVALID_FILE;
    }
    fseek(fp, 0, SEEK_END);
    long size = ftell(fp);
    fseek(fp, 0, SEEK_SET);
    if (size <= 0) { fclose(fp); return MARS_ERR_INVALID_FILE; }
    void *buf = malloc((size_t)size);
    if (!buf) { fclose(fp); return MARS_ERR_ALLOC_FAILED; }
    if (fread(buf, 1, (size_t)size, fp) != (size_t)size) { free(buf); fclose(fp); return MARS_ERR_INVALID_FILE; }
    fclose(fp);
    mars_error_t err = mars_load_memory(buf, (size_t)size, model);
    free(buf);
    return err;
}

mars_runtime_tensor_t *mars_get_input(mars_model_t *model, int index) {
    if (!model || index < 0 || (uint32_t)index >= model->header.num_inputs) return NULL;
    uint32_t tid = model->header.input_tensor_ids[index];
    if (tid >= model->header.num_tensors) return NULL;
    return &model->tensors[tid];
}

mars_runtime_tensor_t *mars_get_output(mars_model_t *model, int index) {
    if (!model || index < 0 || (uint32_t)index >= model->header.num_outputs) return NULL;
    uint32_t tid = model->header.output_tensor_ids[index];
    if (tid >= model->header.num_tensors) return NULL;
    return &model->tensors[tid];
}

int mars_get_num_inputs(mars_model_t *model) { return model ? (int)model->header.num_inputs : 0; }
int mars_get_num_outputs(mars_model_t *model) { return model ? (int)model->header.num_outputs : 0; }

void mars_print_summary(mars_model_t *model) {
    if (!model) return;
    mars_model_ext_t *m = (mars_model_ext_t *)model;
    printf("\nMars model summary (MI355X)\n");
    printf("Layers: %u\n", model->header.num_layers);
    printf("Tensors: %u\n", model->header.num_tensors);
    printf("Inputs: %u\n", model->header.num_inputs);
    printf("Outputs: %u\n", model->header.num_outputs);
    printf("Weights: %zu bytes\n", model->weights_size);
    printf("Launches per run: %d, batch %d, activations %zu bytes, parameters %zu bytes\n\n", m->n_ops, m->batch,
           m->act_bytes, m->arena_size);
}
```

### thingino-accel_amd/csrc/host/mars_plan.c

```c
#include <math.h>
#include <stdio.h>
#include <stdlib.h>
#include <string.h>
#include <time.h>

#include "mars_internal.h"
#include "nna.h"

int32_t mars_trunc_x86(float x) {
    if (x >= -2147483648.0f && x < 2147483648.0f) return (int32_t)x;
    return INT32_MIN;
}
static int sat8(int32_t v) { return v > 127 ? 127 : (v < -128 ? -128 : v); }
static int q_half_up(float v) { return sat8(mars_trunc_x86(v + 0.5f)); }

size_t elem_size(uint32_t dtype) {
    switch (dtype) {
        case MARS_DTYPE_FLOAT32: case MARS_DTYPE_INT32: return 4;
        case MARS_DTYPE_INT16: return 2;
        default: return 1;
    }
}

size_t shape_numel(const mars_tensor_t *d) {
// ... 534 lines not shown
    return 1;
}

static int writer_before(const mars_model_ext_t *m, int t, int before) {
    for (int k = before - 1; k >= 0; k--)
        if (m->ops[k].t_out == t) return k;
    return -1;
}

enum { USE_READ = 1, USE_WRITE = 2 };
static int touched_between(const mars_model_ext_t *m, int lo, int hi, int t, int how) {
    for (int k = lo < 0 ? 0 : lo; k < hi && k < m->n_ops; k++)
        if (((how & USE_READ) && op_reads(&m->ops[k], t)) || ((how & USE_WRITE) && op_writes(&m->ops[k], t))) return 1;
    return 0;
}
static int touched_by_other(const mars_model_ext_t *m, int t, int lo, int hi) {
    return touched_between(m, 0, lo, t, USE_READ | USE_WRITE) || touched_between(m, hi + 1, m->n_ops, t, USE_READ | USE_WRITE);
}

static void drop_dead_ops(mars_model_ext_t *m) {
    int w = 0;
    for (int i = 0; i < m->n_ops; i++)
        if (m->ops[i].kind != -1) m->ops[w++] = m->ops[i];
    m->n_ops = w;
}

size_t planned_stride(const mtensor_t *t) {
    size_t s = ALIGN_UP(t->extent > t->bytes ? t->extent : t->bytes, 256);
    return s ? s : 256;
}

static void lut2_from_lut(mars_model_ext_t *m, mars_op_t *c, const int8_t *tab) {
    if (!mhip_conv_i8_lut2_ok(c->cs)) return;
    int8_t tab2[512];
    for (int k = -256; k < 256; k++) {
        int r = k >= 0 ? (k + 1) >> 1 : -((1 - k) >> 1);
        const int lo = c->relu ? 0 : -128;
        r = r < lo ? lo : (r > 127 ? 127 : r);
        tab2[k + 256] = tab[r + 128];
    }
    c->lut2_off = arena_reserve(m, 512);
    if (c->lut2_off != NO_OFF) memcpy(m->arena_host + c->lut2_off, tab2, 512);
}

void conv_i8_geometry(const mars_op_t *op, int frames, mhip_conv_i8_t *p) {
    memset(p, 0, sizeof(*p));
    p->frames = frames;
    p->in_c = op->in_c; p->in_h = op->in_h; p->in_w = op->in_w;
    p->out_h = op->out_h; p->out_w = op->out_w; p->out_c = op->store_c ? op->store_c : op->out_c;
    p->kh = op->kh; p->kw = op->kw; p->stride_h = op->sh; p->stride_w = op->sw; p->pad_top = op->pt; p->pad_left = op->pl;
    p->row_pad = op->row_pad; p->oc_pad = op->oc_pad; p->safe = op->safe;
    p->out_pix_stride = op->out_pix_stride; p->out_ch_off = op->out_ch_off;
}
int conv_i8_pre_fits(const mars_op_t *op, int frames, size_t in_stride, size_t out_stride) {
    mhip_conv_i8_t p;
    conv_i8_geometry(op, frames, &p);
    p.in_stride = in_stride; p.out_stride = out_stride;
    p.pre_w = (const int8_t *)op; p.pre_bias = (const int32_t *)op; p.pre_lut2 = (const uint8_t *)op; p.lut2 = (const uint8_t *)op;
    p.lut = (const uint8_t *)op;
    return mhip_conv_i8_pre_ok(&p);
}

int conv_i8_post_fits(const mars_model_ext_t *m, const mars_op_t *a, const mars_op_t *b, int frames) {
    mhip_conv_i8_t p;
    if (a->t_in[0] < 0 || a->t_out < 0 || b->t_out < 0) return 0;
    conv_i8_geometry(a, frames, &p);
    p.in_stride = planned_stride(&m->mt[a->t_in[0]]); p.out_stride = planned_stride(&m->mt[a->t_out]);
    p.lut = p.lut2 = p.post_lut2 = (const uint8_t *)a;
    p.post_w = p.post_in = (const int8_t *)a; p.post_out = (int8_t *)m;
    if (a->add_t) p.add = (const int8_t *)a;
    p.post_out_stride = planned_stride(&m->mt[b->t_out]);
    p.post_out_pix_stride = b->out_pix_stride; p.post_out_ch_off = b->out_ch_off;
    return mhip_conv_i8_post_ok(&p);
}

int conv_i8_split_fits(const mars_model_ext_t *m, const mars_op_t *a, const mars_op_t *b, const mars_op_t *c, int frames) {
    mhip_conv_i8_t p;
    if (a->t_in[0] < 0 || a->t_out < 0 || b->t_out < 0 || c->t_out < 0) return 0;
    conv_i8_geometry(a, frames, &p);
    p.in_stride = planned_stride(&m->mt[a->t_in[0]]); p.out_stride = planned_stride(&m->mt[a->t_out]);
    p.lut = p.lut2 = p.split_lut2[0] = p.split_lut2[1] = (const uint8_t *)a;
    p.split_w = (const int8_t *)a; p.split_out[0] = p.split_out[1] = (int8_t *)m;
    p.split_out_stride[0] = planned_stride(&m->mt[b->t_out]); p.split_out_stride[1] = planned_stride(&m->mt[c->t_out]);
    return mhip_conv_i8_split_ok(&p);
}

static int match_silu(const mars_model_ext_t *m, int i, int f32, const int *readers, const int *writers, int q[3], int *fwd) {
    const mars_op_t *c = &m->ops[i], *s = c + 1, *mu = c + 2;
    if (c->kind != (f32 ? OP_CONV_F32 : OP_CONV_I8) || s->kind != (f32 ? OP_SIGMOID_F32 : OP_LUT_I8) || mu->kind != (f32 ? OP_BINARY_F32 : OP_BINARY_I8) || !mu->is_mul)
        return 0;
    if (!f32 && m->pub.layers[s->layer].desc.type != MARS_LAYER_SIGMOID) return 0;
    const int q1 = q[0] = c->t_out, q2 = q[1] = s->t_out, q3 = q[2] = mu->t_out;
    if (s->t_in[0] != q1 || q1 == q2 || q2 == q3 || q1 == q3) return 0;
    *fwd = mu->t_in[0] == q1 && mu->t_in[1] == q2;
    if (!*fwd && !(mu->t_in[0] == q2 && mu->t_in[1] == q1)) return 0;
    if (f32 ? q3 == c->t_in[0] || m->mt[q3].is_weight : op_reads(c, q3)) return 0;
    if (readers[q1] != 2 || readers[q2] != 1 || writers[q1] != 1 || writers[q2] != 1 || writers[q3] != 1) return 0;
    if (m->mt[q1].io_out || m->mt[q2].io_out || m->mt[q1].io_in || m->mt[q2].io_in) return 0;
    const size_t n1 = (size_t)c->out_h * c->out_w * c->out_c;
    return s->n == n1 && mu->n == n1;
}

void fold_silu(mars_model_ext_t *m, int f32) {
    int *readers, *writers;
    if (!use_counts(m, &readers, &writers)) return;
    for (int i = 0; i + 2 < m->n_ops; i++) {
        mars_op_t *c = &m->ops[i];
        int q[3], fwd;
        if (!match_silu(m, i, f32, readers, writers, q, &fwd)) continue;
        const size_t n1 = (size_t)c->out_h * c->out_w * c->out_c;
        if (f32) {
            c->silu_f32 = 1;
        } else {
            const mars_tensor_t *d1 = &m->pub.tensors[q[0]].desc, *d2 = &m->pub.tensors[q[1]].desc, *d3 = &m->pub.tensors[q[2]].desc;
            int8_t tab[256];
            for (int v = -128; v < 128; v++) {
                int sg = sigmoid_q(v, d1->scale, d2->scale);
                tab[v + 128] = (int8_t)(fwd ? binary_q(1, v, sg, d1->scale, d2->scale, d3->scale)
                                            : binary_q(1, sg, v, d2->scale, d1->scale, d3->scale));
            }
            c->lut_off = lut_i8(m, tab);
            lut2_from_lut(m, c, tab);
        }
        c->t_out = q[2];
        touch(m, q[2], n1 * (f32 ? 4 : 1));
        m->mt[q[0]].needed = 0;
        m->mt[q[1]].needed = 0;
        memmove(&m->ops[i + 1], &m->ops[i + 3], (size_t)(m->n_ops - i - 3) * sizeof(mars_op_t));
        m->n_ops -= 2;
    }
    free(readers);
}

void fuse_lut(mars_model_ext_t *m) {
    if (m->sw.no_fuse_lut) return;
    int *readers, *writers;
    if (!use_counts(m, &readers, &writers)) return;
    for (int i = 0; i + 1 < m->n_ops; i++) {
        mars_op_t *c = &m->ops[i], *s = &m->ops[i + 1];
        if (c->kind != OP_CONV_I8 || s->kind != OP_LUT_I8 || c->lut_off != NO_OFF || s->lut_off == NO_OFF) continue;
        const int q1 = c->t_out, q2 = s->t_out;
        if (q1 < 0 || q2 < 0 || s->t_in[0] != q1 || q1 == q2) continue;
        if (op_reads(c, q2)) continue;
        if (readers[q1] != 1 || writers[q1] != 1 || writers[q2] != 1 || m->mt[q1].io_out || m->mt[q1].io_in || m->mt[q1].is_weight || m->mt[q2].is_weight) continue;
        const size_t n1 = (size_t)c->out_h * c->out_w * c->out_c;
        if (s->n != n1 || m->mt[q2].bytes < n1) continue;
        if (m->pub.tensors[q1].desc.dtype != MARS_DTYPE_INT8 || m->pub.tensors[q2].desc.dtype != MARS_DTYPE_INT8) continue;
        c->lut_off = s->lut_off;
        lut2_from_lut(m, c, (const int8_t *)(m->arena_host + s->lut_off));
        c->t_out = q2;
        touch(m, q2, n1);
        m->mt[q1].needed = 0;
        memmove(&m->ops[i + 1], &m->ops[i + 2], (size_t)(m->n_ops - i - 2) * sizeof(mars_op_t));
        m->n_ops -= 1;
    }
    free(readers);
}

void elide_concat(mars_model_ext_t *m) {
    int *readers, *writers;
    if (!use_counts(m, &readers, &writers)) return;
    for (int i = 0; i < m->n_ops; i++) {
        mars_op_t *cs = &m->ops[i];
        if (cs->kind != OP_CONCAT_SLICE) continue;
        const int ti = cs->t_in[0], to = cs->t_out;
        const mtensor_t *mt = &m->mt[ti];
// ... 349 lines not shown
}

void fuse_post(mars_model_ext_t *m) {
    if (m->sw.no_post || m->no_post) return;
    int *readers, *writers;
    if (!use_counts(m, &readers, &writers)) return;
    for (int i = 0; i + 1 < m->n_ops; i++) {
        mars_op_t *a = &m->ops[i], *b = &m->ops[i + 1];
        if (a->kind != OP_CONV_I8 || b->kind != OP_CONV_I8 || a->pre || b->pre || a->post_next || b->post_next || a->pair_next || b->pair_next ||
            (i > 0 && (m->ops[i - 1].pair_next || m->ops[i - 1].post_next)))
            continue;
        const int c = a->out_c, T = a->t_out, O = b->t_out;
        if ((c != 32 && c != 64) || a->oc_pad != c || a->kh * a->kw < 2 || a->sh != 1 || a->sw != 1 || !a->safe || a->nchw || a->out_nchw || a->nseg ||
            a->out_pix_stride || a->out_ch_off || a->store_c || a->chain_n || a->in_byte_off || a->out_byte_off || a->lut_off == NO_OFF ||
            a->lut2_off == NO_OFF || a->n_in >= 4)
            continue;
        if (b->kh != 1 || b->kw != 1 || b->sh != 1 || b->sw != 1 || b->pt || b->pl || !b->safe || b->nchw || b->out_nchw || b->add_t || b->chain_n ||
            b->store_c || b->in_byte_off || b->lut_off == NO_OFF || b->lut2_off == NO_OFF || b->nseg != 2 || b->seg_up || b->seg_t[0] != T ||
            b->seg_c[0] != c || b->seg_c[1] != c || b->in_c != 2 * c || b->out_c != 2 * c || b->oc_pad != 2 * c || b->row_pad != 2 * c ||
            b->in_h != a->out_h || b->in_w != a->out_w || b->out_h != a->out_h || b->out_w != a->out_w)
            continue;
        const int Y = b->seg_t[1];
        if (T < 0 || O < 0 || Y < 0 || Y == T || O == T || O == Y || readers[T] != 1 || writers[T] != 1 || m->mt[T].io_in || m->mt[T].io_out ||
            m->mt[T].is_weight || m->mt[T].tail_read || m->mt[Y].is_weight || m->mt[Y].pix_stride ||
            m->mt[Y].bytes != (size_t)a->out_h * a->out_w * c || op_reads(a, O) || op_reads(a, Y))
            continue;
        if (!conv_i8_post_fits(m, a, b, 1)) continue;
        const size_t bytes = mhip_conv_i8_post_pack(c, NULL, NULL, NULL);
        const size_t off = arena_reserve(m, bytes);
        if (off == NO_OFF) break;
        mhip_conv_i8_post_pack(c, (const int8_t *)(m->arena_host + b->w_off), b->b_off != NO_OFF ? (const int32_t *)(m->arena_host + b->b_off) : NULL,
                               (int8_t *)(m->arena_host + off));
        a->post_next = 1;
        a->post_w_off = off;
        a->t_in[a->n_in++] = Y;
        m->mt[T].needed = 0;
        readers[T] = 0;
        readers[Y]++;
        i++;
    }
    free(readers);
}

static int split_mate_ok(const mars_op_t *b, const mars_op_t *a, int T) {
    return b->kind == OP_CONV_I8 && b->kh == 1 && b->kw == 1 && b->sh == 1 && b->sw == 1 && !b->pt && !b->pl && b->safe && !b->nchw && !b->out_nchw && !b->add_t &&
           !b->chain_n && !b->store_c && !b->in_byte_off && !b->out_byte_off && !b->out_pix_stride && !b->out_ch_off && b->lut_off != NO_OFF &&
           b->lut2_off != NO_OFF && !b->nseg && !b->pre && !b->post_next && !b->split_next && b->n_in == 1 && b->t_in[0] == T && b->in_c == 64 &&
           b->out_c == 32 && b->oc_pad == 32 && b->row_pad == 64 && b->in_h == a->out_h && b->in_w == a->out_w && b->out_h == a->out_h && b->out_w == a->out_w;
}
void fuse_split(mars_model_ext_t *m) {
    if (m->sw.no_split || m->no_split) return;
    int *readers, *writers;
    if (!use_counts(m, &readers, &writers)) return;
    for (int i = 0; i + 2 < m->n_ops; i++) {
        mars_op_t *a = &m->ops[i], *b = &m->ops[i + 1], *c = &m->ops[i + 2];
        if (a->kind != OP_CONV_I8 || a->pre || a->post_next || a->split_next || a->pair_next || !b->pair_next || c->pair_next ||
            (i > 0 && (m->ops[i - 1].pair_next || m->ops[i - 1].post_next)))
            continue;
        const int T = a->t_out;
        if (a->out_c != 64 || a->oc_pad != 64 || a->kh * a->kw < 2 || (a->sh != 1 && a->sh != 2) || a->sw != a->sh || !a->safe || a->nchw || a->out_nchw ||
            a->nseg || a->out_pix_stride || a->out_ch_off || a->store_c || a->chain_n || a->in_byte_off || a->out_byte_off || a->add_t ||
            a->lut_off == NO_OFF || a->lut2_off == NO_OFF || a->n_in != 1)
            continue;
        if (T < 0 || !split_mate_ok(b, a, T) || !split_mate_ok(c, a, T)) continue;
        const int O0 = b->t_out, O1 = c->t_out;
        if (O0 < 0 || O1 < 0 || O0 == O1 || O0 == T || O1 == T || readers[T] != 2 || writers[T] != 1 || m->mt[T].io_in || m->mt[T].io_out ||
            m->mt[T].is_weight || m->mt[T].tail_read || m->mt[O0].pix_stride || m->mt[O1].pix_stride || op_reads(a, O0) || op_reads(a, O1))
            continue;
        if (!conv_i8_split_fits(m, a, b, c, 1)) continue;
        const size_t bytes = mhip_conv_i8_split_pack(NULL, NULL, NULL, NULL, NULL);
        const size_t off = arena_reserve(m, bytes);
        if (off == NO_OFF) break;
        mhip_conv_i8_split_pack((const int8_t *)(m->arena_host + b->w_off), b->b_off != NO_OFF ? (const int32_t *)(m->arena_host + b->b_off) : NULL,
                                (const int8_t *)(m->arena_host + c->w_off), c->b_off != NO_OFF ? (const int32_t *)(m->arena_host + c->b_off) : NULL,
                                (int8_t *)(m->arena_host + off));
        a->split_next = 1;
        a->split_w_off = off;
        m->mt[T].needed = 0;
        i += 2;
    }
    free(readers);
}

void pad_output_rows(mars_model_ext_t *m) {
    for (uint32_t i = 0; i < m->pub.header.num_tensors; i++) m->mt[i].pix_c = m->mt[i].pix_stride = 0;
    if (m->sw.no_rowpad) return;
    for (int i = 0; i < m->n_ops; i++) {
        mars_op_t *o = &m->ops[i];
        if (o->kind != OP_CONV_I8 || o->out_nchw || o->out_pix_stride || o->out_ch_off || o->add_t || o->t_out < 0 ||
            (o->out_c & 15) == 0 || (o->in_c & 15) != 0)
            continue;
        mtensor_t *t = &m->mt[o->t_out];
        const int P = (o->out_c + 15) & ~15;
        const size_t px = (size_t)o->out_h * o->out_w;
        if (!t->io_out || t->io_in || P > o->oc_pad || t->bytes != px * (size_t)o->out_c || (px * P) % 256 != 0) continue;
        if (touched_by_other(m, o->t_out, i, i)) continue;
        o->out_pix_stride = P;
        o->store_c = P;
        t->pix_c = o->out_c;
        t->pix_stride = P;
        if (px * P > t->extent) t->extent = px * P;
    }
}

void virtual_concat(mars_model_ext_t *m) {
    const int nt = (int)m->pub.header.num_tensors;
    for (int T = 0; T < nt; T++) {
        const mtensor_t *mt = &m->mt[T];
        if (mt->is_weight || mt->io_in || mt->io_out) continue;
        int sl[4], ns = 0, bad = 0, first_reader = -1, last_reader = -1, last_slice = -1;
        for (int i = 0; i < m->n_ops && !bad; i++) {
            const mars_op_t *o = &m->ops[i];
            if (o->t_out == T) {
                if (o->kind != OP_CONCAT_SLICE || ns >= 4) bad = 1;
                else { sl[ns++] = i; last_slice = i; }
            }
            for (int k = 0; k < o->n_in; k++)
                if (o->t_in[k] == T) {
                    if (o->kind != OP_CONV_I8 || k != 0 || o->n_in != 1 || o->nchw || o->kh != 1 || o->kw != 1 || o->sh != 1 ||
                        o->sw != 1 || o->pt || o->pl || !o->safe || o->nseg || (o->out_c & 15) || o->in_h != o->out_h ||
                        o->in_w != o->out_w || (o->in_c & (o->in_c - 1)) != 0 || o->add_t)
                        bad = 1;
                    if (first_reader < 0) first_reader = i;
                    last_reader = i;
                }
        }
        if (bad || ns < 2 || first_reader < 0 || last_slice > first_reader) continue;
        for (int a = 0; a < ns; a++)
            for (int b = a + 1; b < ns; b++)
                if (m->ops[sl[b]].ch_off < m->ops[sl[a]].ch_off) { int t = sl[a]; sl[a] = sl[b]; sl[b] = t; }
        int c = 0;
        const mars_op_t *s0 = &m->ops[sl[0]];
        for (int a = 0; a < ns && !bad; a++) {
            const mars_op_t *o = &m->ops[sl[a]];
            if (o->ch_off != c || (o->in_c & 31) || o->out_h != s0->out_h || o->out_w != s0->out_w || o->out_c != s0->out_c ||
                o->t_in[0] == T || o->t_in[0] < 0)
                bad = 1;
            c += o->in_c;
            if (!bad && touched_between(m, sl[a] + 1, last_reader + 1, o->t_in[0], USE_WRITE)) bad = 1;
        }
        if (bad || c != s0->out_c) continue;
        for (int i = 0; i < m->n_ops && !bad; i++) {
            const mars_op_t *o = &m->ops[i];
            if (o->kind == OP_CONV_I8 && o->n_in == 1 && o->t_in[0] == T &&
                (o->in_c != c || (size_t)o->in_h * o->in_w != (size_t)s0->out_h * s0->out_w))
                bad = 1;
        }
        if (bad) continue;
        for (int i = 0; i < m->n_ops; i++) {
            mars_op_t *o = &m->ops[i];
            if (o->kind != OP_CONV_I8 || o->n_in != 1 || o->t_in[0] != T) continue;
            o->nseg = ns;
            o->n_in = ns;
            for (int a = 0; a < ns; a++) {
                o->seg_t[a] = o->t_in[a] = m->ops[sl[a]].t_in[0];
                o->seg_c[a] = m->ops[sl[a]].in_c;
            }
        }
        for (int a = 0; a < ns; a++) m->ops[sl[a]].kind = -1;
        m->mt[T].needed = 0;
        for (int a = 0; a < ns; a++) {
            const int S = m->ops[sl[a]].t_in[0];
            int up = -1, nread = 0, nwrite = 0, ok = 1;
            for (int i = 0; i < m->n_ops; i++) {
                const mars_op_t *o = &m->ops[i];
                if (o->kind == -1) continue;
// ... 309 lines not shown
            if (!m->deferred)
                mhip_conv_f32_vcat_pack(x->out_c, x->in_c, (int)km + 1, (const float *)(m->arena_host + x->w_off), (float *)(m->arena_host + wt_off[q]));
        }
        while (m->n_ops + heads > m->cap_ops) {
            const int cap = m->cap_ops * 2;
            mars_op_t *np = (mars_op_t *)realloc(m->ops, (size_t)cap * sizeof(mars_op_t));
            if (!np) { m->plan_err = MARS_ERR_ALLOC_FAILED; return; }
            m->ops = np; m->cap_ops = cap;
        }
        memmove(&m->ops[rl + 1 + heads], &m->ops[rl + 1], sizeof(mars_op_t) * (size_t)(m->n_ops - rl - 1));
        m->n_ops += heads;
        for (int q = 0; q < heads; q++) {
            mars_op_t *x = &m->ops[r1 + q], *h = &m->ops[rl + 1 + q];
            const double hw = (double)x->in_h * x->in_w;
            x->t_in[0] = TL;
            x->vc_shift = (int)sB;
            x->k_limit = (int)km;
            x->macs = hw * x->out_c * (double)km;
            x->bytes = (hw * (double)km + hw * x->out_c) * 4.0;
            *h = *x;
            h->kind = OP_CONV_F32_VHEAD;
            h->pair_next = 0; h->vc_shift = 0;
            h->k_limit = (int)km + 1;
            h->vc_n = N - 1; h->vc_run = Wb / 4;
            h->n_in = N;
            for (int k = 0; k < N - 1; k++) { h->vc_t[k] = firsts[k]; h->t_in[1 + k] = firsts[k]; }
            h->macs = (double)(sB / 4) * x->out_c * (double)(km + 1);
            h->bytes = ((double)(sB / 4) * (double)(km + 1) + (double)(sB / 4) * x->out_c) * 4.0;
            h->variant = 0;
            h->w3_off = wt_off[q]; h->w3_stem = 0;
            h->w2_off = NO_OFF; h->w2_planes = 0;
        }
        memmove(&m->ops[first_op], &m->ops[e + 1], sizeof(mars_op_t) * (size_t)(m->n_ops - e - 1));
        m->n_ops -= N;
        m->mt[T].needed = 0;
        m->mt[T].partial = 1;
        m->mt[T].zero_from = 0;
        i = first_op - 1;
    }
}

void f32_policy(mars_model_ext_t *m) {
    const int nt = (int)m->pub.header.num_tensors;
    unsigned char *hot = (unsigned char *)calloc((size_t)nt + 1, 1);
    if (!hot) {
        for (int i = 0; i < m->n_ops; i++) m->ops[i].f32_exact = 1;
        return;
    }
    for (int i = m->n_ops - 1; i >= 0; i--) {
        mars_op_t *o = &m->ops[i];
        int reach = 0;
        if (o->kind == OP_MAXPOOL && o->t_in[0] >= 0 && m->pub.tensors[o->t_in[0]].desc.dtype == MARS_DTYPE_FLOAT32) reach = 1;
        if (o->kind == OP_RELU_BYTES && o->t_out >= 0) {
            hot[o->t_out] = 1;
            continue;
        }
        if (o->t_out >= 0 && hot[o->t_out]) reach = 1;
        for (int k = 0; k < o->chain_n; k++)
            if (o->chain_out[k] >= 0 && hot[o->chain_out[k]]) reach = 1;
        if (!reach) continue;
        for (int k = 0; k < o->n_in; k++)
            if (o->t_in[k] >= 0) hot[o->t_in[k]] = 1;
        if (o->kind == OP_CONV_F32) o->f32_exact = 1;
    }
    free(hot);
}

void plan_check(mars_model_ext_t *m) {
    for (int i = 0; i < m->n_ops; i++) {
        const mars_op_t *o = &m->ops[i];
        const char *why = NULL;
        if (o->kind == -1) why = "a dead op is left";
        else if (o->n_in < 0 || o->n_in > 4 || o->nseg < 0 || o->nseg > 4 || o->chain_n < 0 || o->chain_n > 3 || o->vc_n < 0 || o->vc_n > 3) why = "an operand count is out of range";
        else if (o->add_t && !op_reads(o, o->add_t - 1)) why = "add_t is not among t_in";
        else if (o->chain_n && o->t_out != o->chain_out[o->chain_n - 1]) why = "t_out is not the chain's last stage";
        else if (o->pair_next && (i + 1 >= m->n_ops || m->ops[i + 1].kind != o->kind)) why = "pair_next without a mate of its kind";
        else if (o->post_next && (o->kind != OP_CONV_I8 || i + 1 >= m->n_ops || m->ops[i + 1].kind != OP_CONV_I8 || m->ops[i + 1].nseg != 2 ||
                                  m->ops[i + 1].seg_t[0] != o->t_out || !op_reads(o, m->ops[i + 1].seg_t[1])))
            why = "post_next without its 1x1 behind it, or y2 is not among t_in";
        else if (o->split_next && (o->kind != OP_CONV_I8 || i + 2 >= m->n_ops || m->ops[i + 1].kind != OP_CONV_I8 || m->ops[i + 2].kind != OP_CONV_I8 ||
                                   !m->ops[i + 1].pair_next || m->ops[i + 2].pair_next || m->ops[i + 1].n_in != 1 || m->ops[i + 2].n_in != 1 ||
                                   m->ops[i + 1].t_in[0] != o->t_out || m->ops[i + 2].t_in[0] != o->t_out || o->post_next || o->pair_next || o->pre || o->add_t))
            why = "split_next without its pair of 1x1s behind it";
        for (int k = 0; !why && k < o->nseg; k++)
            if (!op_reads(o, o->seg_t[k])) why = "a seg_t is not among t_in";
        for (int k = 0; !why && k < o->vc_n; k++)
            if (!op_reads(o, o->vc_t[k])) why = "a vc_t is not among t_in";
        if (!why) continue;
        VLOG("plan_check: op %d (layer %d, kind %d): %s\n", i, o->layer, o->kind, why);
        m->plan_err = MARS_ERR_LAYER_FAILED;
        return;
    }
}
```

### thingino-accel_amd/csrc/host/mars_run.c

```c
#include <math.h>
#include <stdio.h>
#include <stdlib.h>
#include <string.h>
#include <time.h>

#include "mars_internal.h"
#include "nna.h"

static int g_graph_max_batch = 8;
static unsigned g_tune_gen = 1;
static int g_dual_min_batch = 64;
static int g_dual_ways = 2;
static uint8_t *tdev(const mars_model_ext_t *m, int ti) {
    if (ti < 0 || !m->mt[ti].dev) return NULL;
    return m->mt[ti].dev + (m->mt[ti].is_weight ? 0 : (size_t)m->frame0 * m->mt[ti].stride);
}
static size_t tstride(const mars_model_ext_t *m, int ti) { return ti >= 0 ? m->mt[ti].stride : 0; }

void conv_i8_params(const mars_model_ext_t *m, const mars_op_t *op, mhip_conv_i8_t *p) {
    uint8_t *A = m->arena_dev;
    conv_i8_geometry(op, m->run_frames, p);
    p->in = (const int8_t *)tdev(m, op->t_in[0]); p->in_stride = tstride(m, op->t_in[0]);
    p->out = (int8_t *)tdev(m, op->t_out); p->out_stride = tstride(m, op->t_out);
    if (p->in) p->in += op->in_byte_off;
    if (p->out) p->out += op->out_byte_off;
    p->w = (const int8_t *)(A + op->w_off);
    p->bias = op->b_off != NO_OFF ? (const int32_t *)(A + op->b_off) : NULL;
    p->lut = op->lut_off != NO_OFF ? A + op->lut_off : NULL;
    p->lut2 = op->lut_off != NO_OFF && op->lut2_off != NO_OFF ? A + op->lut2_off : NULL;
    p->w_rgb = op->w2_off != NO_OFF && !op->w2_rows ? (const int8_t *)(A + op->w2_off) : NULL;
    p->w_rows = op->w2_off != NO_OFF && op->w2_rows ? (const int8_t *)(A + op->w2_off) : NULL;
    if (op->pre) {
        p->pre_w = (const int8_t *)(A + op->pre_w_off);
        p->pre_bias = (const int32_t *)(A + op->pre_b_off);
        p->pre_lut2 = A + op->pre_lut2_off;
        p->pre_cs = op->pre_cs;
    }
    p->cs = op->cs; p->relu = op->relu; p->out_nchw = op->out_nchw;
    p->variant = op->variant;
    if ((op->post_next || op->split_next) && op->t_out >= 0) p->out_stride = planned_stride(&m->mt[op->t_out]);
    if (op->add_t && tstride(m, op->add_t - 1) == p->out_stride) {
        p->add = (const int8_t *)tdev(m, op->add_t - 1);
        p->add_s_conv = op->add_s_conv; p->add_s_other = op->add_s_other; p->add_inv = op->add_inv;
    }
    p->nseg = op->nseg;
    p->seg_up = op->seg_up;
    int c0 = 0;
    for (int k = 0; k < 4; k++) {
        p->seg_c0[k] = 0x7fffffff;
        if (k < op->nseg) {
            p->seg_in[k] = (const int8_t *)tdev(m, op->seg_t[k]);
            p->seg_stride[k] = tstride(m, op->seg_t[k]);
            p->seg_c[k] = op->seg_c[k];
            p->seg_c0[k] = c0;
            c0 += op->seg_c[k];
        }
    }
    if (op->nseg > 1) p->in = p->seg_in[0];
}

static void conv_i8_post_params(const mars_model_ext_t *m, const mars_op_t *op, const mars_op_t *cv3, mhip_conv_i8_t *p) {
    uint8_t *A = m->arena_dev;
    conv_i8_params(m, op, p);
    p->post_w = (const int8_t *)(A + op->post_w_off);
    p->post_lut2 = A + cv3->lut2_off;
    p->post_cs = cv3->cs;
    p->post_in = (const int8_t *)tdev(m, cv3->seg_t[1]); p->post_in_stride = tstride(m, cv3->seg_t[1]);
    p->post_out = (int8_t *)tdev(m, cv3->t_out); p->post_out_stride = tstride(m, cv3->t_out);
    if (p->post_out) p->post_out += cv3->out_byte_off;
    p->post_out_pix_stride = cv3->out_pix_stride; p->post_out_ch_off = cv3->out_ch_off;
}

static void conv_i8_split_params(const mars_model_ext_t *m, const mars_op_t *op, const mars_op_t *cv1, const mars_op_t *cv2, mhip_conv_i8_t *p) {
    uint8_t *A = m->arena_dev;
    const mars_op_t *side[2] = {cv1, cv2};
    conv_i8_params(m, op, p);
    p->split_w = (const int8_t *)(A + op->split_w_off);
    for (int k = 0; k < 2; k++) {
        p->split_lut2[k] = A + side[k]->lut2_off;
        p->split_cs[k] = side[k]->cs;
        p->split_out[k] = (int8_t *)tdev(m, side[k]->t_out); p->split_out_stride[k] = tstride(m, side[k]->t_out);
    }
}

static void conv_f32_params(mars_model_ext_t *m, mars_op_t *op, mhip_conv_f32_t *p) {
    const int B = m->run_frames;
    uint8_t *A = m->arena_dev;
    memset(p, 0, sizeof(*p));
    p->in = (const float *)tdev(m, op->t_in[0]); p->in_stride = tstride(m, op->t_in[0]);
    p->out = (float *)tdev(m, op->t_out); p->out_stride = tstride(m, op->t_out);
    p->w = (const float *)(A + op->w_off);
    p->w_split = op->w2_off != NO_OFF ? (const void *)(A + op->w2_off) : NULL;
    p->w_patch = op->w3_off != NO_OFF ? (const void *)(A + op->w3_off) : NULL;
    p->bias = op->b_off != NO_OFF ? (const float *)(A + op->b_off) : NULL;
    p->frames = B;
    p->in_h = op->in_h; p->in_w = op->in_w; p->in_c = op->in_c;
    p->out_h = op->out_h; p->out_w = op->out_w; p->out_c = op->out_c;
    p->kh = op->kh; p->kw = op->kw; p->stride_h = op->sh; p->stride_w = op->sw; p->pad_top = op->pt; p->pad_left = op->pl;
    p->silu = op->silu_f32;
    if (op->add_t) { p->add = (const float *)tdev(m, op->add_t - 1); p->add_stride = tstride(m, op->add_t - 1); }
    {
        const int mode = mhip_conv_f32_mode(-1);
        p->use_mfma = mode == 3 ? 3 : mode == 4 ? 2 : (mode == 2 || (mode == 1 && !op->f32_exact));
    }
    if (op->in_rec || op->out_rec) {
        p->in_rec = op->in_rec; p->out_rec = op->out_rec;
        p->use_mfma = 3;
    }
    {
        const int need = p->use_mfma == 2 ? 3 : p->use_mfma == 3 ? 2 : 0;
        if (need > op->w2_planes) p->w_split = NULL;
        if (p->use_mfma != 3) p->w_patch = NULL;
    }
    if (p->use_mfma >= 2) p->k_limit = op->k_limit;
    if (op->vc_shift && op->kind == OP_CONV_F32) {
        p->in = p->in ? (const float *)((const uint8_t *)p->in - op->vc_shift) : NULL;
        p->k_limit = op->k_limit;
        p->k_limit_required = 1;
        if (p->use_mfma < 2 || !p->w_split) p->in = NULL;
    }
}

static int launch_op(mars_model_ext_t *m, mars_op_t *op) {
    const int B = m->run_frames;
    uint8_t *A = m->arena_dev;
    switch (op->kind) {
        case OP_CONV_I8: {
            mhip_conv_i8_t p;
            conv_i8_params(m, op, &p);
            if (op->nchw && op->c_pad == 4 && op->in_c <= 4 && !op->add_t) {
                if (!getenv("MARS_HIP_NO_PLANAR_STEM")) {
                    mhip_conv_i8_t q = p;
                    q.in_c = op->c_pad;
                    q.in_planar = op->in_c;
                    const int rc = mhip_conv_i8(&q);
                    if (rc != -2) return rc;
                }
            }
            if (op->nchw) {
                const size_t ss = ALIGN_UP(m->scratch_per_frame, 256);
                int8_t *scratch = (int8_t *)m->scratch_dev + (size_t)m->frame0 * ss;
                if (!(m->scratch_t == op->t_in[0] && m->scratch_cpad == op->c_pad && m->scratch_f0 == m->frame0 && m->scratch_n == B)) {
                    int rc = mhip_nchw_to_nhwc_pad(p.in, p.in_stride, scratch, ss, B, op->in_c, op->in_h * op->in_w, op->c_pad);
                    if (rc) return rc;
                    m->scratch_t = op->t_in[0]; m->scratch_cpad = op->c_pad; m->scratch_f0 = m->frame0; m->scratch_n = B;
                }
                p.in = scratch; p.in_stride = ss; p.in_c = op->c_pad;
            }
            if (op->add_t && !p.add) return -1;
            return mhip_conv_i8(&p);
        }
        case OP_CONV_F32: {
            mhip_conv_f32_t p;
            conv_f32_params(m, op, &p);
            return mhip_conv_f32(&p);
        }
        case OP_CONV_F32_VHEAD: {
            mhip_conv_f32_t p;
            const float *first[3] = {NULL, NULL, NULL};
            size_t strides[3] = {0, 0, 0};
            conv_f32_params(m, op, &p);
            if (p.use_mfma < 2) return -1;
            p.k_limit = op->k_limit;
            for (int k = 0; k < op->vc_n && k < 3; k++) {
                first[k] = (const float *)tdev(m, op->vc_t[k]);
// ... 82 lines not shown
    }
}

static mars_error_t enqueue_plan(mars_model_t *model);
static double now_us(void);
static int tune_raw(const char *key, int value, int *get);

static void tune_push(mars_model_ext_t *m) {
    if (m->tune_depth++ || !m->n_tune) return;
    for (int i = 0; i < m->n_tune; i++) {
        tune_raw(m->tune[i].key, 0, &m->tune[i].saved);
        tune_raw(m->tune[i].key, m->tune[i].value, NULL);
    }
}
static void tune_pop(mars_model_ext_t *m) {
    if (--m->tune_depth || !m->n_tune) return;
    for (int i = m->n_tune - 1; i >= 0; i--) tune_raw(m->tune[i].key, m->tune[i].saved, NULL);
}
static mars_error_t run_device_async(mars_model_t *model);
mars_error_t mars_hip_run_device_async(mars_model_t *model) {
    if (!model) return MARS_ERR_INVALID_FILE;
    tune_push((mars_model_ext_t *)model);
    mars_error_t e = run_device_async(model);
    tune_pop((mars_model_ext_t *)model);
    return e;
}

static mars_error_t run_device_async(mars_model_t *model) {
    mars_model_ext_t *m = (mars_model_ext_t *)model;
    if (!m->act_dev || !m->arena_dev) return MARS_ERR_NNA_INIT_FAILED;
    int graphable = g_graph_max_batch > 0 && m->batch <= g_graph_max_batch && !m->profiling && !m->pipe;
    for (int i = 0; i < m->n_ops && graphable; i++)
        if (m->ops[i].kind == OP_FAIL) graphable = 0;
    if (!graphable) return enqueue_plan(model);
    if (m->graph_exec && m->graph_gen != g_tune_gen) {
        drop_graph(m);
        m->ran_plain = 0;
    }
    if (!m->graph_exec) {
        if (!m->ran_plain) {
            mars_error_t e = enqueue_plan(model);
            if (e == MARS_OK) m->ran_plain = 1;
            return e;
        }
        if (m->tail_pending) {
            mhip_select_stream(0);
            if (mhip_stream_wait(0, m->ev_tail_done)) return MARS_ERR_LAYER_FAILED;
            m->tail_pending = 0;
        }
        if (mhip_graph_begin() == 0) {
            mars_error_t e = enqueue_plan(model);
            m->graph_exec = mhip_graph_end(e == MARS_OK);
            m->graph_gen = g_tune_gen;
            if (e != MARS_OK) { m->graph_exec = NULL; return e; }
        }
        VLOG("plan of %d launches at batch %d %s\n", m->n_ops, m->batch, m->graph_exec ? "captured into a HIP graph" : "could not be captured");
        if (!m->graph_exec) {
            g_graph_max_batch = 0;
            return enqueue_plan(model);
        }
    }
    if (m->tail_pending) {
        mhip_select_stream(0);
        if (mhip_stream_wait(0, m->ev_tail_done)) return MARS_ERR_LAYER_FAILED;
        m->tail_pending = 0;
    }
    if (mhip_graph_launch(m->graph_exec)) return MARS_ERR_LAYER_FAILED;
    for (uint32_t i = 0; i < model->header.num_layers; i++) model->layers[i].is_executed = true;
    return MARS_OK;
}

static mars_error_t enqueue_range(mars_model_ext_t *m, int sid, int wait_tail) {
    void *prof_last = NULL;
    mhip_select_stream(sid);
    m->scratch_t = -1;
    for (int i = 0; i < m->n_ops; i++) {
        mars_op_t *op = &m->ops[i];
        if (op->kind == OP_FAIL) {
            fprintf(stderr, "Mars: Layer %d execution failed\n", op->layer);
            return (mars_error_t)op->err;
        }
        mars_op_t *mate = (op->pair_next || op->post_next || op->split_next) && i + 1 < m->n_ops ? &m->ops[i + 1] : NULL;
        mars_op_t *mate2 = op->split_next && i + 2 < m->n_ops ? &m->ops[i + 2] : NULL;
        if (wait_tail && ((op->t_out >= 0 && (m->mt[op->t_out].io_out || m->mt[op->t_out].tail_read)) ||
                          (mate && mate->t_out >= 0 && (m->mt[mate->t_out].io_out || m->mt[mate->t_out].tail_read)) ||
                          (mate2 && mate2->t_out >= 0 && (m->mt[mate2->t_out].io_out || m->mt[mate2->t_out].tail_read)))) {
            mhip_stream_wait(sid, m->ev_tail_done);
            wait_tail = 0;
        }
        if (m->profiling) {
            if (!op->ev1) op->ev1 = mhip_event_create();
            if (!prof_last) {
                if (!op->ev0) op->ev0 = mhip_event_create();
                mhip_event_record(op->ev0);
                prof_last = op->ev0;
            }
            op->ev_start = prof_last;
        }
        int rc;
        if (op->split_next) {
            mhip_conv_i8_t pa;
            rc = -1;
            if (mate && mate2) {
                conv_i8_split_params(m, op, mate, mate2, &pa);
                rc = mhip_conv_i8(&pa);
            }
            i += 2;
        } else if (mate && op->post_next) {
            mhip_conv_i8_t pa;
            conv_i8_post_params(m, op, mate, &pa);
            rc = mhip_conv_i8(&pa);
            i++;
        } else if (mate && op->kind == OP_CONV_F32) {
            mhip_conv_f32_t pa, pb;
            conv_f32_params(m, op, &pa);
            conv_f32_params(m, mate, &pb);
            rc = mhip_conv_f32_pair(&pa, &pb);
            if (rc == -2) {
                rc = launch_op(m, op);
                if (!rc) rc = launch_op(m, mate);
            }
            i++;
        } else if (mate) {
            mhip_conv_i8_t pa, pb;
            conv_i8_params(m, op, &pa);
            conv_i8_params(m, mate, &pb);
            rc = mhip_conv_i8_pair(&pa, &pb);
            if (rc == -2) {
                rc = launch_op(m, op);
                if (!rc) rc = launch_op(m, mate);
            }
            i++;
        } else {
            rc = launch_op(m, op);
        }
        {
            const mars_op_t *w2[3] = {op, mate, mate2};
            for (int q = 0; q < 3; q++)
                if (w2[q] && op_writes(w2[q], m->scratch_t)) m->scratch_t = -1;
        }
        if (m->profiling) {
            const int nx = i + 1;
            const int end = m->profiling != 2 || nx >= m->n_ops || m->ops[nx].prof_kind != op->prof_kind;
            op->prof_rec = end;
            if (end) {
                mhip_event_record(op->ev1);
                prof_last = op->ev1;
            }
        }
        if (rc != 0) {
            fprintf(stderr, "Mars: Layer %d launch failed: %s\n", op->layer, mhip_last_error());
            return MARS_ERR_LAYER_FAILED;
        }
    }
    return MARS_OK;
}

static mars_error_t enqueue_plan(mars_model_t *model) {
    mars_model_ext_t *m = (mars_model_ext_t *)model;
    for (uint32_t i = 0; i < model->header.num_layers; i++) model->layers[i].is_executed = false;
    const int B = m->batch;
    int dual = g_dual_min_batch > 0 && B >= g_dual_min_batch && B >= 2 && !m->profiling &&
               !(g_graph_max_batch > 0 && B <= g_graph_max_batch);
    if (dual) {
        if (!m->ev_fork) m->ev_fork = mhip_event_create_sync();
        for (int k = 0; k < 3; k++) {
            if (!m->ev_join[k]) m->ev_join[k] = mhip_event_create_sync();
            if (!m->ev_join[k]) dual = 0;
        }
        if (!m->ev_fork) dual = 0;
    }
    mars_error_t e;
    if (!dual) {
        m->frame0 = 0; m->run_frames = B;
        e = enqueue_range(m, 0, m->tail_pending);
    } else {
        const int ways = g_dual_ways < B ? g_dual_ways : B;
        mhip_select_stream(0);
        int rc = mhip_event_record(m->ev_fork);
        for (int k = 1; k < ways && !rc; k++) rc = mhip_stream_wait(3 + k, m->ev_fork);
        if (rc) return MARS_ERR_LAYER_FAILED;
        e = MARS_OK;
        int f0 = 0;
        for (int k = 0; k < ways && e == MARS_OK; k++) {
            const int n = (B - f0 + (ways - k) - 1) / (ways - k);
            m->frame0 = f0; m->run_frames = n;
            e = enqueue_range(m, k ? 3 + k : 0, m->tail_pending);
            f0 += n;
        }
        for (int k = 1; k < ways; k++) {
            mhip_select_stream(3 + k);
            rc = mhip_event_record(m->ev_join[k - 1]);
            if (!rc) rc = mhip_stream_wait(0, m->ev_join[k - 1]);
            if (rc && e == MARS_OK) e = MARS_ERR_LAYER_FAILED;
        }
    }
    mhip_select_stream(0);
    m->frame0 = 0; m->run_frames = B;
    if (e != MARS_OK) return e;
    m->tail_pending = 0;
    for (uint32_t i = 0; i < model->header.num_layers; i++) model->layers[i].is_executed = true;
    return MARS_OK;
}

static double now_us(void) {
    struct timespec ts;
    clock_gettime(CLOCK_MONOTONIC, &ts);
    return ts.tv_sec * 1e6 + ts.tv_nsec * 1e-3;
}

mars_error_t mars_hip_run_device(mars_model_t *model) {
    double t0 = now_us();
    mars_error_t e = mars_hip_run_device_async(model);
    if (e != MARS_OK) { mhip_sync(); return e; }
    if (mhip_sync()) return MARS_ERR_LAYER_FAILED;
    mars_model_ext_t *m = (mars_model_ext_t *)model;
    if (m->profiling)
        for (int i = 0; i < m->n_ops; i++)
            m->ops[i].last_ms = (m->ops[i].prof_rec && m->ops[i].ev_start && m->ops[i].ev1) ? mhip_event_elapsed_ms(m->ops[i].ev_start, m->ops[i].ev1) : 0.f;
    model->total_inference_us += (uint64_t)(now_us() - t0);
    model->inference_count++;
// ... 175 lines not shown
        return 0;
    }
    return get ? mhip_conv_i8_tune_get(key, get) : mhip_conv_i8_tune(key, value);
}

static mars_error_t replan_for_f32_mode(mars_model_ext_t *m) {
    if (m->deferred || !m->arena_dev) return MARS_OK;
    int has_f32 = 0;
    for (int i = 0; i < m->n_ops && !has_f32; i++) has_f32 = m->ops[i].kind == OP_CONV_F32;
    if (!has_f32) return MARS_OK;
    tune_push(m);
    const int mode = mhip_conv_f32_mode(-1);
    mars_error_t e = MARS_OK;
    if (mode != m->plan_f32_mode && (mode >= 3 || m->plan_f32_mode >= 3)) {
        mhip_sync();
        e = build_plan(m);
        if (e == MARS_OK) e = upload_params(m);
        if (e == MARS_OK) e = alloc_batch(m, m->batch > 0 ? m->batch : 1);
    }
    tune_pop(m);
    return e;
}

int mars_hip_set_tuning(const char *key, int value) {
    g_tune_gen++;
    int rc = tune_raw(key, value, NULL);
    if (rc == 0 && key && !strcmp(key, "f32_mfma"))
        for (mars_model_ext_t *m = mars_live_models(); m; m = m->live_next)
            if (replan_for_f32_mode(m) != MARS_OK) rc = -1;
    return rc;
}

int mars_hip_get_tuning(const char *key, int *value) { return value ? tune_raw(key, 0, value) : -1; }

int mars_hip_model_set_tuning(mars_model_t *model, const char *key, int value) {
    mars_model_ext_t *m = (mars_model_ext_t *)model;
    int cur;
    if (!m || !key || strlen(key) >= sizeof m->tune[0].key || tune_raw(key, 0, &cur)) return -1;
    if (tune_raw(key, value, NULL)) return -1;
    tune_raw(key, cur, NULL);
    int i = 0;
    while (i < m->n_tune && strcmp(m->tune[i].key, key)) i++;
    if (i == m->n_tune) {
        if (m->n_tune == MARS_MAX_MODEL_TUNE) return -1;
        strcpy(m->tune[m->n_tune++].key, key);
    }
    m->tune[i].value = value;
    drop_graph(m);
    if (!strcmp(key, "f32_mfma") && replan_for_f32_mode(m) != MARS_OK) return -1;
    return 0;
}

int mars_hip_model_get_tuning(mars_model_t *model, const char *key, int *value) {
    mars_model_ext_t *m = (mars_model_ext_t *)model;
    if (!m || !key || !value) return -1;
    for (int i = 0; i < m->n_tune; i++)
        if (!strcmp(m->tune[i].key, key)) { *value = m->tune[i].value; return 0; }
    return tune_raw(key, 0, value);
}

static mars_error_t autotune_model(mars_model_t *model, int reps);
mars_error_t mars_hip_autotune(mars_model_t *model, int reps) {
    if (!model) return MARS_ERR_INVALID_FILE;
    tune_push((mars_model_ext_t *)model);
    mars_error_t e = autotune_model(model, reps);
    tune_pop((mars_model_ext_t *)model);
    return e;
}
static mars_error_t autotune_model(mars_model_t *model, int reps) {
    mars_model_ext_t *m = (mars_model_ext_t *)model;
    if (!m->act_dev || !m->arena_dev) return MARS_ERR_NNA_INIT_FAILED;
    drop_graph(m);
    if (reps <= 0) reps = 3;
    void *e0 = mhip_event_create(), *e1 = mhip_event_create();
    if (!e0 || !e1) return MARS_ERR_ALLOC_FAILED;
    mars_error_t err = MARS_OK;
    if (mhip_sync()) err = MARS_ERR_LAYER_FAILED;
    for (int i = 0; i < m->n_ops && err == MARS_OK; i++) {
        mars_op_t *op = &m->ops[i];
        if (op->kind != OP_CONV_I8 || op->nchw) continue;
        if (op->pair_next || (i > 0 && m->ops[i - 1].pair_next)) continue;
        if (op->post_next || (i > 0 && m->ops[i - 1].post_next)) continue;
        if (op->split_next) continue;
        mhip_conv_i8_t p;
        conv_i8_params(m, op, &p);
        int codes[32];
        const int n = mhip_conv_i8_variants(&p, codes, 32);
        if (getenv("MARS_VERBOSE") && atoi(getenv("MARS_VERBOSE")) > 1)
            fprintf(stderr, "Mars: autotune layer %d: %dx%dx%d -> %dx%dx%d k%dx%d s%d pixstride %d choff %d lut %d safe %d\n", op->layer,
                    p.in_h, p.in_w, p.in_c, p.out_h, p.out_w, p.out_c, p.kh, p.kw, p.stride_w, p.out_pix_stride, p.out_ch_off,
                    p.lut != NULL, p.safe);
        float best = 0.0f;
        int best_code = 0;
        for (int k = 0; k < n && err == MARS_OK; k++) {
            p.variant = codes[k];
            int rc = mhip_conv_i8(&p);
            if (!rc) rc = mhip_event_record(e0);
            for (int r = 0; r < reps && !rc; r++) rc = mhip_conv_i8(&p);
            if (!rc) rc = mhip_event_record(e1);
            if (rc || mhip_sync()) { err = MARS_ERR_LAYER_FAILED; break; }
            const float ms = mhip_event_elapsed_ms(e0, e1);
            if (getenv("MARS_VERBOSE") && atoi(getenv("MARS_VERBOSE")) > 1)
                fprintf(stderr, "Mars: autotune layer %d: candidate %d: %.1f us\n", op->layer, codes[k], ms * 1000.0f / reps);
            if (best_code == 0 || ms < best) { best = ms; best_code = codes[k]; }
        }
        if (err == MARS_OK && best_code) {
            if (getenv("MARS_VERBOSE"))
                fprintf(stderr, "Mars: autotune layer %d: variant %d (%.1f us) of %d candidates, default %d\n", op->layer,
                        best_code, best * 1000.0f / reps, n, n ? codes[0] : 0);
            op->variant = best_code;
        }
    }
    mhip_event_destroy(e0);
    mhip_event_destroy(e1);
    return err;
}

void *mars_hip_tensor_device(mars_model_t *model, int ti, size_t *frame_stride) {
    if (!model || ti < 0 || (uint32_t)ti >= model->header.num_tensors) return NULL;
    mars_model_ext_t *m = (mars_model_ext_t *)model;
    if (frame_stride) *frame_stride = m->mt[ti].stride;
    return m->mt[ti].dev;
}

size_t mars_hip_tensor_frame_bytes(const mars_model_t *model, int ti) {
    if (!model || ti < 0 || (uint32_t)ti >= model->header.num_tensors) return 0;
    return ((const mars_model_ext_t *)model)->mt[ti].bytes;
}

int mars_hip_tensor_row_pitch(mars_model_t *model, int ti, int *row_bytes) {
    if (!model || ti < 0 || (uint32_t)ti >= model->header.num_tensors) return 0;
    const mtensor_t *t = &((mars_model_ext_t *)model)->mt[ti];
    if (row_bytes) *row_bytes = t->pix_stride ? t->pix_c : 0;
    return t->pix_stride;
}

mars_error_t mars_hip_read_tensor(mars_model_t *model, int ti, int frame, void *dst, size_t bytes) {
    if (!model || !dst || ti < 0 || (uint32_t)ti >= model->header.num_tensors) return MARS_ERR_INVALID_TENSOR;
    mars_model_ext_t *m = (mars_model_ext_t *)model;
    mtensor_t *t = &m->mt[ti];
    if (!t->dev || frame < 0 || (!t->is_weight && frame >= m->batch)) return MARS_ERR_INVALID_TENSOR;
    if (!t->is_weight && bytes > t->stride) return MARS_ERR_INVALID_TENSOR;
    if (t->partial) return MARS_ERR_INVALID_TENSOR;
    if (t->is_weight) {
        const size_t off = (size_t)m->pub.tensors[ti].desc.data_offset;
        if (off > m->blob_mirror_bytes || bytes > m->blob_mirror_bytes - off) return MARS_ERR_INVALID_TENSOR;
        frame = 0;
    }
    if (mhip_sync()) return MARS_ERR_LAYER_FAILED;
    if (t->rec_c) {
        const size_t full = (size_t)t->rec_c * t->rec_hw * 4;
        uint8_t *raw = (uint8_t *)malloc(full);
        float *f = (float *)malloc(full);
        if (!raw || !f || bytes > full || mhip_d2h_async(raw, t->dev + (size_t)frame * t->stride, full) || mhip_sync()) {
            free(raw); free(f);
            return MARS_ERR_LAYER_FAILED;
        }
        for (int c = 0; c < t->rec_c; c++)
            for (int px = 0; px < t->rec_hw; px++) {
                const uint8_t *r = raw + ((size_t)(c >> 3) * t->rec_hw + px) * 32 + (size_t)(c & 7) * 2;
                uint16_t h, md;
                memcpy(&h, r, 2); memcpy(&md, r + 16, 2);
                const uint32_t hb = (uint32_t)h << 16, mb = (uint32_t)md << 16;
                float hf, mf;
                memcpy(&hf, &hb, 4); memcpy(&mf, &mb, 4);
                f[(size_t)c * t->rec_hw + px] = hf + mf;
// ... 120 lines not shown
```

### thingino-accel_amd/csrc/mhip.h

```cpp
#ifndef MHIP_H
#define MHIP_H

#include <stddef.h>
#include <stdint.h>

#ifdef __cplusplus
extern "C" {
#endif

int mhip_init(int device_hint);
void mhip_shutdown(void);
int mhip_ready(void);
int mhip_device_info(int *cu_count, int *lds_bytes, int *gfx_version, size_t *hbm_bytes);
void *mhip_stream(void);
int mhip_sync(void);
void mhip_select_aux(int on);
void mhip_select_stream(int which);
int mhip_stream_wait(int which, void *ev);
int mhip_event_sync(void *ev);
void *mhip_malloc(size_t bytes);
void mhip_free(void *p);
void *mhip_host_alloc(size_t bytes);
void mhip_host_free(void *p);
int mhip_memset_async(void *dst, int value, size_t bytes);
int mhip_h2d_async(void *dst, const void *src, size_t bytes);
int mhip_d2h_async(void *dst, const void *src, size_t bytes);
int mhip_d2d_async(void *dst, const void *src, size_t bytes);
int mhip_h2d_2d_async(void *dst, size_t dpitch, const void *src, size_t spitch, size_t row_bytes, size_t rows);
int mhip_d2h_2d_async(void *dst, size_t dpitch, const void *src, size_t spitch, size_t row_bytes, size_t rows);
void *mhip_event_create(void);
void *mhip_event_create_sync(void);
void mhip_event_destroy(void *ev);
int mhip_event_record(void *ev);
float mhip_event_elapsed_ms(void *start, void *stop);
const char *mhip_last_error(void);
int mhip_graph_begin(void);
void *mhip_graph_end(int ok);
int mhip_graph_launch(void *exec);
void mhip_graph_destroy(void *exec);

typedef struct {
    const int8_t *in;  size_t in_stride;
    int8_t *out;       size_t out_stride;
    const int8_t *w;
    const int32_t *bias;
    const uint8_t *lut;
    const uint8_t *lut2;
    const int8_t *pre_w;
    const int32_t *pre_bias;
    const uint8_t *pre_lut2;
    float pre_cs;
    const int8_t *w_rgb;
    const int8_t *w_rows;
    int frames;
    int in_h, in_w, in_c;
    int out_h, out_w, out_c;
    int kh, kw, stride_h, stride_w, pad_top, pad_left;
    int row_pad;
    int oc_pad;
    float cs;
    int relu;
    int out_nchw;
    int in_planar;
    int safe;
    int out_pix_stride;
    int out_ch_off;
    int variant;
    const int8_t *add;
    float add_s_conv, add_s_other, add_inv;
    int nseg;
    const int8_t *seg_in[4];
    size_t seg_stride[4];
    int seg_c[4], seg_c0[4];
    int seg_up;
    const int8_t *post_w;
    const uint8_t *post_lut2;
    float post_cs;
    const int8_t *post_in;  size_t post_in_stride;
    int8_t *post_out;       size_t post_out_stride;
    int post_out_pix_stride, post_out_ch_off;
    const int8_t *split_w;
    const uint8_t *split_lut2[2];
    float split_cs[2];
    int8_t *split_out[2];   size_t split_out_stride[2];
} mhip_conv_i8_t;
int mhip_conv_i8_split_ok(const mhip_conv_i8_t *p);
size_t mhip_conv_i8_split_pack(const int8_t *packed0, const int32_t *bias0, const int8_t *packed1, const int32_t *bias1, int8_t *out);
int mhip_conv_i8_split_row(int side, int oc);
int mhip_conv_i8_post_ok(const mhip_conv_i8_t *p);
size_t mhip_conv_i8_post_pack(int c, const int8_t *packed, const int32_t *bias, int8_t *out);
int mhip_conv_i8_post_k(int c, int k);
int mhip_conv_i8_post_row(int c, int oc);
int mhip_conv_i8_oc_row(int oc, int oc_pad);
int mhip_conv_i8_pre_ok(const mhip_conv_i8_t *p);
size_t mhip_conv_i8_rgb_pack(int in_c, int kh, int kw, int stride_h, int stride_w, int pad_left, int oc_pad, int k64,
                             const int8_t *packed, int8_t *out);
size_t mhip_conv_i8_rows_pack(int in_c, int kh, int kw, int stride_h, int stride_w, int oc_pad, int k64, int out_w,
                              const int8_t *packed, int8_t *out);
unsigned long mhip_conv_i8_rows_launches(void);
int mhip_conv_i8_is_safe(float cs);
int mhip_conv_i8_lut2_ok(float cs);
int mhip_conv_i8_tune(const char *key, int value);
int mhip_conv_i8_tune_get(const char *key, int *value);
int mhip_conv_i8_variants(const mhip_conv_i8_t *p, int *codes, int max);
int mhip_conv_i8_seg_ok(const mhip_conv_i8_t *p);
int mhip_conv_i8_pair(const mhip_conv_i8_t *a, const mhip_conv_i8_t *b);
int mhip_conv_i8_small_c(int in_c, int kw, int out_c);
void mhip_conv_i8_pack_geom(int in_c, int kw, int out_c, int *row_pad, int *oc_pad, int *c_eff);
int mhip_conv_i8(const mhip_conv_i8_t *p);

typedef struct {
    const float *in;  size_t in_stride;
    float *out;       size_t out_stride;
    const float *w;   const float *bias;
    const void *w_split;
    const void *w_patch;
    int frames;
    int in_h, in_w, in_c, out_h, out_w, out_c;
    int kh, kw, stride_h, stride_w, pad_top, pad_left;
    int silu;
    const float *add; size_t add_stride;
    int use_mfma;
    int k_limit;
    int k_limit_required;
    int in_rec, out_rec;
} mhip_conv_f32_t;
int mhip_conv_f32(const mhip_conv_f32_t *p);
size_t mhip_conv_f32_vcat_pack(int out_c, int in_c, int planes, const float *w, float *out);
int mhip_conv_f32_vcat_head(const mhip_conv_f32_t *p, const float *w_t, const float *const *first, const size_t *first_strides, int n_first, int run_floats);
int mhip_conv_f32_pair(const mhip_conv_f32_t *a, const mhip_conv_f32_t *b);
unsigned long mhip_conv_f32_pair_launches(void);
size_t mhip_conv_f32_split_pack(int out_c, int in_c, int kh, int kw, int stride_w, int planes, const float *w, void *out);
unsigned long mhip_conv_f32_split_launches(void);
int mhip_conv_f32_split_takes(int out_c, int in_c, int kh, int kw, int stride_h, int stride_w, int pad_left, int in_w, int out_w);
size_t mhip_conv_f32_patch_pack(int out_c, int in_c, int kh, int kw, int stride, int pad, int in_h, int in_w, int out_h, int out_w,
                                const float *w, void *out);
size_t mhip_conv_f32_patch_pack2(int out_c, int in_c, int kh, int kw, int stride, int pad, int in_h, int in_w, int out_h, int out_w,
                                 int rec, const float *w, void *out);
int mhip_conv_f32_patch_geom2(int out_c, int in_c, int kh, int kw, int stride, int pad, int in_h, int in_w, int out_h, int out_w,
                              int rec, int *outv, int cap);
unsigned long mhip_conv_f32_prec_launches(void);
unsigned long mhip_conv_f32_recin_launches(void);
int mhip_conv_f32_patch_rec_form(int out_c, int in_c, int kh, int kw, int stride, int pad, int in_h, int in_w, int out_h, int out_w);
int mhip_conv_f32_patch_geom(int out_c, int in_c, int kh, int kw, int stride, int pad, int in_h, int in_w, int out_h, int out_w,
                             int *outv, int cap);
unsigned long mhip_conv_f32_patch_launches(void);
size_t mhip_conv_f32_stem_pack(int out_c, int in_c, int kh, int kw, int stride, int pad, int in_h, int in_w, int out_h, int out_w,
                               const float *w, void *out);
unsigned long mhip_conv_f32_stem_launches(void);
int mhip_conv_f32_mode(int set);

int mhip_lut_i8(const int8_t *in, size_t in_stride, int8_t *out, size_t out_stride, int frames,
                size_t n, const uint8_t *lut_dev);
int mhip_relu_bytes(int8_t *buf, size_t stride, int frames, size_t n);
int mhip_binary_i8(int is_mul, const int8_t *a, size_t a_stride, const int8_t *b, size_t b_stride,
                   int8_t *out, size_t out_stride, int frames, size_t n, float sa, float sb, float inv_so,
                   int out_run, int out_pix_stride, int out_ch_off);
int mhip_sigmoid_f32(const float *in, size_t in_stride, float *out, size_t out_stride, int frames, size_t n);
int mhip_binary_f32(int op , const float *a, size_t a_stride, const float *b,
                    size_t b_stride, float *out, size_t out_stride, int frames, size_t n);
int mhip_relu_f32(const float *in, size_t in_stride, float *out, size_t out_stride, int frames,
                  size_t n, float alpha);
int mhip_batchnorm_i8(const int8_t *in, size_t in_stride, int8_t *out, size_t out_stride, int frames,
                      int n, int c, int hw, const float *s, const float *b, float in_scale, float out_scale);
int mhip_batchnorm_f32(const float *in, size_t in_stride, float *out, size_t out_stride, int frames,
                       int n, int c, int hw, const float *s, const float *b);

int mhip_maxpool_i8(const int8_t *in, size_t in_stride, int8_t *out, size_t out_stride, int frames,
                    int in_h, int in_w, int ch, int out_h, int out_w, int kh, int kw, int sh, int sw,
                    int out_pix_stride, int out_ch_off);
int mhip_pool_chain_i8(const int8_t *in, size_t in_stride, int8_t *const *outs, const size_t *out_strides, int n,
// ... 257 lines not shown
```

Before: 60490.

## Fuse a following 32-channel 1x1 conv into the split-conv patch kernel

Extends the SPLIT patch kernel with a CHAIN stage: the requantized output of one split side is fed straight into an extra 32x32 1x1 conv via MFMA inside the same kernel, then requantized through a third LUT and stored. The host planner finds a matching 1x1 op within a window, reorders it next to the split pair, packs its weights, and launches one kernel instead of two. This removes a launch and a global round trip of the intermediate activation, at the cost of more LDS use, which may lower occupancy, plus extra register pressure in the tail.

```diff
diff --git a/thingino-accel_amd/csrc/hip/conv_i8_common.hpp b/thingino-accel_amd/csrc/hip/conv_i8_common.hpp
--- a/thingino-accel_amd/csrc/hip/conv_i8_common.hpp
+++ b/thingino-accel_amd/csrc/hip/conv_i8_common.hpp
@@ -188,6 +188,26 @@
 #pragma unroll
     for (int g = 0; g < 4; g++) pk[g] = pack4(v[4 * g], v[4 * g + 1], v[4 * g + 2], v[4 * g + 3]);
 }
+__device__ __forceinline__ void requant_pack_chain(const int (&a)[8], float cs, uint32_t (&pk)[2]) {
+    const float cs2 = cs * 2.0f;
+    const int klo = -256, khi = 255;
+    int q[8], v[8];
+#pragma unroll
+    for (int i = 0; i < 8; i++) {
+        const int k = (int)((float)a[i] * cs2);
+        asm("v_med3_i32 %0, %1, %2, %3" : "=v"(q[i]) : "v"(k), "v"(klo), "v"(khi));
+    }
+#pragma unroll
+    for (int g = 0; g < 2; g++)
+        asm volatile("ds_read_i8 %0, %4 offset:1792\n\tds_read_i8 %1, %5 offset:1792\n\t"
+                     "ds_read_i8 %2, %6 offset:1792\n\tds_read_i8 %3, %7 offset:1792"
+                     : "=&v"(v[4 * g]), "=&v"(v[4 * g + 1]), "=&v"(v[4 * g + 2]), "=&v"(v[4 * g + 3])
+                     : "v"(q[4 * g]), "v"(q[4 * g + 1]), "v"(q[4 * g + 2]), "v"(q[4 * g + 3])
+                     : "memory");
+    wait_lds_values<8>(v);
+#pragma unroll
+    for (int g = 0; g < 2; g++) pk[g] = pack4(v[4 * g], v[4 * g + 1], v[4 * g + 2], v[4 * g + 3]);
+}
 template <int NV, bool HAS_LUT, bool SAFE, bool LUT0, bool ADD = false, bool FAST = false>
 __device__ __forceinline__ void requant_pack(const int (&a)[NV], float cs, int lo, const uint8_t *lut128, uint32_t (&pk)[NV / 4],
                                              const uint32_t *xw = nullptr, const add_args_t *ga = nullptr) {
diff --git a/thingino-accel_amd/csrc/hip/conv_i8_patch.hip b/thingino-accel_amd/csrc/hip/conv_i8_patch.hip
--- a/thingino-accel_amd/csrc/hip/conv_i8_patch.hip
+++ b/thingino-accel_amd/csrc/hip/conv_i8_patch.hip
@@ -41,7 +41,7 @@
     asm volatile("s_waitcnt lgkmcnt(0)\n\ts_barrier" ::: "memory");
 }
 
-template <int TH, int BN, bool HAS_LUT, bool PRE = false, bool POST = false, bool SPLIT = false>
+template <int TH, int BN, bool HAS_LUT, bool PRE = false, bool POST = false, bool SPLIT = false, bool CHAIN = false>
 __global__ __launch_bounds__(NTHREADS) void conv_i8_patch(const mhip_conv_i8_t p, const int k64, const int tiles_x,
                                                           const int tiles_y, const unsigned ntiles_all, const int PH,
                                                           const int PW, const int PWP, const int PWH, const int nblk,
@@ -58,7 +58,8 @@
     const int nks = k64 / BK;
     constexpr int NPO = 2 * BN;
     static_assert(!SPLIT || (BN == 64 && HAS_LUT && !PRE && !POST), "SPLIT: one 64-channel tile, no other stage");
-    constexpr int LB = LUTB + ((PRE || POST) ? 512 : 0) + (SPLIT ? 1024 : 0);
+    static_assert(!CHAIN || SPLIT, "CHAIN: a stage of the SPLIT form");
+    constexpr int LB = LUTB + ((PRE || POST) ? 512 : 0) + (SPLIT ? 1024 : 0) + (CHAIN ? 512 : 0);
     int *dutab = (int *)(dynlds + LB);
     int8_t *wl = dynlds + LB + ((nks * 16 + 255) & ~255);
     const int patch_bytes = nblk * 1024;
@@ -67,7 +68,9 @@
     const int *pbl = (const int *)(pwl + NPO * NPO);
     int8_t *swl = w1l;
     const int *sbl = (const int *)(swl + 64 * BK);
-    int8_t *patch0 = w1l + (PRE ? p.in_c * BK : 0) + (POST ? NPO * NPO + NPO * 4 : 0) + (SPLIT ? 64 * BK + 64 * 4 : 0);
+    int8_t *cwl = swl + 64 * BK + 64 * 4;
+    const int *cbl = (const int *)(cwl + 32 * BK);
+    int8_t *patch0 = w1l + (PRE ? p.in_c * BK : 0) + (POST ? NPO * NPO + NPO * 4 : 0) + (SPLIT ? 64 * BK + 64 * 4 : 0) + (CHAIN ? 32 * BK + 32 * 4 : 0);
     int8_t *tpatch = patch0 + ring * patch_bytes;
 
     const int tid = threadIdx.x, lane = tid & 63;
@@ -101,6 +104,10 @@
             ((uint32_t *)slut)[tid + 128] = ((const uint32_t *)p.split_lut2[1])[tid - 128];
         }
         if (tid < 64) ((int *)(swl + 64 * BK))[tid] = ((const int *)(p.split_w + 64 * BK))[tid];
+    }
+    if (CHAIN) {
+        if (tid >= 128) ((uint32_t *)slut)[tid + 256] = ((const uint32_t *)p.chain_lut2)[tid - 128];
+        if (tid >= 64 && tid < 96) ((int *)(cwl + 32 * BK))[tid - 64] = ((const int *)(p.chain_w + 32 * BK))[tid - 64];
     }
     const int rowbytes = p.kw * C, kbytes = p.kh * rowbytes;
     for (int i = tid; i < nks * 4; i += NTHREADS) {
@@ -126,6 +133,8 @@
             for (int i = wv; i < NPO * NPO / 1024; i += 4) glds16(p.post_w + i * 1024 + lane * 16, pwl + i * 1024);
         if (SPLIT)
             glds16(p.split_w + wv * 1024 + lane * 16, swl + wv * 1024);
+        if (CHAIN && wv < 2)
+            glds16(p.chain_w + wv * 1024 + lane * 16, cwl + wv * 1024);
     }
     int uoff[PT_NIMAX], upos[PT_NIMAX];
 #pragma unroll
@@ -184,6 +193,9 @@
     const __amdgpu_buffer_rsrc_t orsrc = __builtin_amdgcn_make_buffer_rsrc(SPLIT ? p.split_out[0] : (POST ? p.post_out : p.out), 0, (int)out_bytes, 0x00020000);
     const unsigned out_bytes1 = SPLIT ? (unsigned)(p.frames - 1) * (unsigned)p.split_out_stride[1] + (unsigned)(p.out_h * p.out_w) * 32u : 0u;
     const __amdgpu_buffer_rsrc_t orsrc1 = __builtin_amdgcn_make_buffer_rsrc(SPLIT ? p.split_out[1] : p.out, 0, (int)out_bytes1, 0x00020000);
+    const unsigned out_bytes2 = CHAIN ? (unsigned)(p.frames - 1) * (unsigned)p.chain_out_stride + (unsigned)(p.out_h * p.out_w) * 32u : 0u;
+    const __amdgpu_buffer_rsrc_t orsrc2 = __builtin_amdgcn_make_buffer_rsrc(CHAIN ? p.chain_out : p.out, 0, (int)out_bytes2, 0x00020000);
+    const bool cside1 = CHAIN && p.chain_side == 2;
     const bool has_add = !SPLIT && p.add != nullptr;
     constexpr int RROW = WOC == 4 ? 1024 : 512;
     constexpr int NRI = WOC == 4 ? WPX : 2 * WPX;
@@ -191,7 +203,7 @@
     const int frow = lane & 15, fchunk = lane >> 4;
     const int chan = (lane >> 4) * (4 * WOC);
     const int NR = has_add || POST ? NRI : 0;
-    const int ntail = POST ? (has_add ? NRI : 0) + WPX * (NPO / 64) : (SPLIT ? 2 * WPX : NST);
+    const int ntail = POST ? (has_add ? NRI : 0) + WPX * (NPO / 64) : (SPLIT ? (CHAIN ? 3 : 2) * WPX : NST);
     const int ppstride = p.post_out_pix_stride ? p.post_out_pix_stride : NPO;
     auto issue_rows = [&](const int8_t *base, size_t fstride, int tx, int ty, unsigned f) {
 #pragma unroll
@@ -474,6 +486,7 @@
                 for (int r = 0; r < 4; r++) sc[u][r] = __builtin_amdgcn_mfma_i32_16x16x64_i8(sw4[r], b0, sb4[r], 0, 0, 0);
             }
             const unsigned fo0 = f * (unsigned)p.split_out_stride[0], fo1 = f * (unsigned)p.split_out_stride[1];
+            uint32_t ck[CHAIN ? WPX : 1][2];
 #pragma unroll
             for (int u = 0; u < WPX; u++) {
                 int a2[16];
@@ -486,6 +499,38 @@
                 const int voff0 = voffs[u] >= 0 ? voffs[u] + (int)fo0 : -1, voff1 = voffs[u] >= 0 ? voffs[u] + (int)fo1 : -1;
                 __builtin_amdgcn_raw_buffer_store_b64((v2i){(int)pk4[0], (int)pk4[1]}, orsrc, voff0, 0, 0);
                 __builtin_amdgcn_raw_buffer_store_b64((v2i){(int)pk4[2], (int)pk4[3]}, orsrc1, voff1, 0, 0);
+                if (CHAIN) {
+                    ck[CHAIN ? u : 0][0] = cside1 ? pk4[2] : pk4[0];
+                    ck[CHAIN ? u : 0][1] = cside1 ? pk4[3] : pk4[1];
+                }
+            }
+            if (CHAIN) {
+                v4i cw4[2], cb4[2];
+#pragma unroll
+                for (int r = 0; r < 2; r++) {
+                    cw4[r] = *(const v4i *)(cwl + lds_off(r * 16 + frow, fchunk));
+                    cb4[r] = *(const v4i *)(cbl + r * 16 + fchunk * 4);
+                }
+                v4i cc[WPX][2];
+#pragma unroll
+                for (int u = 0; u < WPX; u++) {
+                    const v4i b0 = {(int)ck[CHAIN ? u : 0][0], (int)ck[CHAIN ? u : 0][1], 0, 0};
+#pragma unroll
+                    for (int r = 0; r < 2; r++) cc[u][r] = __builtin_amdgcn_mfma_i32_16x16x64_i8(cw4[r], b0, cb4[r], 0, 0, 0);
+                }
+                const unsigned fo2 = f * (unsigned)p.chain_out_stride;
+#pragma unroll
+                for (int u = 0; u < WPX; u++) {
+                    int a1[8];
+#pragma unroll
+                    for (int r = 0; r < 2; r++)
+#pragma unroll
+                        for (int e = 0; e < 4; e++) a1[r * 4 + e] = cc[u][r][e];
+                    uint32_t pk2[2];
+                    requant_pack_chain(a1, p.chain_cs, pk2);
+                    const int voff2 = voffs[u] >= 0 ? voffs[u] + (int)fo2 : -1;
+                    __builtin_amdgcn_raw_buffer_store_b64((v2i){(int)pk2[0], (int)pk2[1]}, orsrc2, voff2, 0, 0);
+                }
             }
         }
         if (POST) {
@@ -586,10 +631,16 @@
         for (int i = 0; i < 2; i++)
             if ((long)(p->frames - 1) * (long)p->split_out_stride[i] + (long)p->out_h * p->out_w * 32 > 0x7fffffffL) return false;
     }
+    const bool chain = p->chain_side != 0;
+    if (chain) {
+        if (!split || (p->chain_side != 1 && p->chain_side != 2) || !p->chain_w || !p->chain_lut2 || !p->chain_out || p->chain_out == p->split_out[0] ||
+            p->chain_out == p->split_out[1] || (long)(p->frames - 1) * (long)p->chain_out_stride + (long)p->out_h * p->out_w * 32 > 0x7fffffffL)
+            return false;
+    }
     const size_t pb = (size_t)g->nblk * 1024;
     const size_t radd = p->add || post ? (size_t)4 * (th / 4) * (g->bn == 64 ? 1024 : 512) : 0;
     const size_t fixed = LUTB + (pre ? 512 + (size_t)C * BK + pb : 0) + (post ? 512 + (size_t)4 * g->bn * g->bn + (size_t)8 * g->bn : 0) +
-                         (split ? 1024 + (size_t)64 * BK + 64 * 4 : 0) +
+                         (split ? 1024 + (size_t)64 * BK + 64 * 4 : 0) + (chain ? 512 + (size_t)32 * BK + 32 * 4 : 0) +
                          (((size_t)g->nks * 16 + 255) & ~(size_t)255) + (size_t)g->nks * g->bn * BK + radd;
     const size_t budget = patch_lds_budget(g->bn);
     if (fixed + pb > budget) return false;
@@ -609,9 +660,9 @@
 static inline long split_out_bytes(const mhip_conv_i8_t *p, int side) {
     return (long)(p->frames - 1) * (long)p->split_out_stride[side] + (long)p->out_h * p->out_w * 32;
 }
-template <int TH, int BN, bool HAS_LUT, bool PRE = false, bool POST = false, bool SPLIT = false>
+template <int TH, int BN, bool HAS_LUT, bool PRE = false, bool POST = false, bool SPLIT = false, bool CHAIN = false>
 static int launch_patch_t(const mhip_conv_i8_t *p, int k64, const patch_geom_t &g) {
-    auto kern = conv_i8_patch<TH, BN, HAS_LUT, PRE, POST, SPLIT>;
+    auto kern = conv_i8_patch<TH, BN, HAS_LUT, PRE, POST, SPLIT, CHAIN>;
     static int cus = 0;
     static size_t slots_lds[8];
     static int slots_n[8], nslots = 0;
@@ -673,6 +724,11 @@
     (p->post_w ? launch_patch_t<T, B, true, false, true>(p, k64, g)                       \
      : p->pre_w ? launch_patch_t<T, B, true, true>(p, k64, g)                             \
                 : (p->lut ? launch_patch_t<T, B, true>(p, k64, g) : launch_patch_t<T, B, false>(p, k64, g)))
+    if (p->split_w && p->chain_side) {
+        if (th == 16) return launch_patch_t<16, 64, true, false, false, true, true>(p, k64, g);
+        if (th == 8) return launch_patch_t<8, 64, true, false, false, true, true>(p, k64, g);
+        return launch_patch_t<4, 64, true, false, false, true, true>(p, k64, g);
+    }
     if (p->split_w) {
         if (th == 16) return launch_patch_t<16, 64, true, false, false, true>(p, k64, g);
         if (th == 8) return launch_patch_t<8, 64, true, false, false, true>(p, k64, g);
@@ -759,3 +815,19 @@
     }
     return bytes;
 }
+
+extern "C" int mhip_conv_i8_chain_k(int c) { return (c >> 3) * 16 + (c & 7); }
+extern "C" size_t mhip_conv_i8_chain_pack(const int8_t *packed, const int32_t *bias, int8_t *out) {
+    const size_t bytes = (size_t)32 * BK + (size_t)32 * 4;
+    if (!packed || !out) return bytes;
+    memset(out, 0, bytes);
+    for (int oc = 0; oc < 32; oc++) {
+        const int R = mhip_conv_i8_split_row(0, oc), src = mhip_conv_i8_oc_row(oc, 32);
+        for (int c = 0; c < 32; c++) {
+            const int k = mhip_conv_i8_chain_k(c);
+            out[(size_t)R * BK + ((((k >> 4) ^ ((R >> 1) & 2))) << 4) + (k & 15)] = packed[(size_t)src * 64 + c];
+        }
+        ((int32_t *)(out + (size_t)32 * BK))[R] = bias ? bias[src] : 0;
+    }
+    return bytes;
+}
diff --git a/thingino-accel_amd/csrc/host/mars_internal.h b/thingino-accel_amd/csrc/host/mars_internal.h
--- a/thingino-accel_amd/csrc/host/mars_internal.h
+++ b/thingino-accel_amd/csrc/host/mars_internal.h
@@ -81,6 +81,8 @@
     size_t post_w_off;
     int split_next;
     size_t split_w_off;
+    int split_chain;
+    size_t chain_w_off;
     size_t w2_off;
     int w2_rows;
     int w2_planes;
@@ -100,7 +102,7 @@
 typedef struct {
     int fusion;
     unsigned no_fuse_lut : 1, no_nhwc_internal : 1, no_vconcat_q : 1, no_pair_f32 : 1, no_rec : 1, no_zero_tail : 1, no_vconcat_f32 : 1,
-        no_rowpad : 1, no_post : 1, no_split : 1;
+        no_rowpad : 1, no_post : 1, no_split : 1, no_chain : 1;
     size_t rec_limit;
     size_t vconcat_limit;
     size_t bottleneck_limit;
@@ -116,6 +118,7 @@
     int no_bottleneck;
     int no_post;
     int no_split;
+    int no_chain;
     int rec_frames;
     int rec_skipped;
     size_t rec_max_frames;
@@ -227,6 +230,7 @@
 MARS_INTERNAL int conv_i8_pre_fits(const mars_op_t *op, int frames, size_t in_stride, size_t out_stride);
 MARS_INTERNAL int conv_i8_post_fits(const mars_model_ext_t *m, const mars_op_t *a, const mars_op_t *b, int frames);
 MARS_INTERNAL int conv_i8_split_fits(const mars_model_ext_t *m, const mars_op_t *a, const mars_op_t *b, const mars_op_t *c, int frames);
+MARS_INTERNAL int conv_i8_chain_fits(const mars_model_ext_t *m, const mars_op_t *a, const mars_op_t *b, const mars_op_t *c, const mars_op_t *d, int side, int frames);
 MARS_INTERNAL void plan_layer(mars_model_ext_t *m, int li);
 MARS_INTERNAL void fold_silu(mars_model_ext_t *m, int f32);
 MARS_INTERNAL void fuse_lut(mars_model_ext_t *m);
@@ -240,6 +244,7 @@
 MARS_INTERNAL void fuse_bottleneck(mars_model_ext_t *m);
 MARS_INTERNAL void fuse_post(mars_model_ext_t *m);
 MARS_INTERNAL void fuse_split(mars_model_ext_t *m);
+MARS_INTERNAL void fuse_split_chain(mars_model_ext_t *m);
 MARS_INTERNAL void pad_output_rows(mars_model_ext_t *m);
 MARS_INTERNAL void virtual_concat_q(mars_model_ext_t *m);
 MARS_INTERNAL void f32_policy(mars_model_ext_t *m);
diff --git a/thingino-accel_amd/csrc/host/mars_model.c b/thingino-accel_amd/csrc/host/mars_model.c
--- a/thingino-accel_amd/csrc/host/mars_model.c
+++ b/thingino-accel_amd/csrc/host/mars_model.c
@@ -28,6 +28,7 @@
     sw->no_rowpad = getenv("MARS_HIP_NO_ROWPAD") != NULL;
     sw->no_post = getenv("MARS_HIP_NO_POST") != NULL;
     sw->no_split = getenv("MARS_HIP_NO_SPLIT") != NULL;
+    sw->no_chain = getenv("MARS_HIP_NO_CHAIN") != NULL;
     sw->rec_limit = (e = getenv("MARS_HIP_REC_LIMIT")) ? (size_t)strtoull(e, NULL, 0) : (size_t)0xfffffff0u;
     sw->vconcat_limit = (e = getenv("MARS_HIP_VCONCAT_LIMIT")) ? (size_t)strtoull(e, NULL, 0) : (size_t)0x7fffffffu;
     sw->bottleneck_limit = (e = getenv("MARS_HIP_BOTTLENECK_LIMIT")) ? (size_t)strtoull(e, NULL, 0) : 0;
@@ -164,6 +165,7 @@
         if (m->sw.fusion >= 2 && !m->no_bottleneck) fuse_bottleneck(m);
         fuse_post(m);
         fuse_split(m);
+        fuse_split_chain(m);
         pad_output_rows(m);
         virtual_concat_q(m);
     } else {
@@ -205,8 +207,8 @@
     const size_t vlim = m->sw.vconcat_limit, blim = m->sw.bottleneck_limit;
     const int rec_replan = (size_t)n > m->rec_max_frames || (m->rec_skipped && n < m->rec_frames);
     m->rec_frames = n;
-    if (m->no_vconcat || m->no_bottleneck || m->no_post || m->no_split || rec_replan) {
-        m->no_vconcat = m->no_bottleneck = m->no_post = m->no_split = 0;
+    if (m->no_vconcat || m->no_bottleneck || m->no_post || m->no_split || m->no_chain || rec_replan) {
+        m->no_vconcat = m->no_bottleneck = m->no_post = m->no_split = m->no_chain = 0;
         mars_error_t e = build_plan(m);
         if (e == MARS_OK) e = upload_params(m);
         if (e != MARS_OK) return e;
@@ -242,6 +244,18 @@
             if (op->kind != OP_CONV_I8 || !op->post_next) continue;
             if (!conv_i8_post_fits(m, op, op + 1, n)) {
                 m->no_post = 1;
+                mars_error_t e = build_plan(m);
+                if (e == MARS_OK) e = upload_params(m);
+                if (e != MARS_OK) return e;
+                break;
+            }
+        }
+    if (!m->no_chain)
+        for (int i = 0; i + 3 < m->n_ops; i++) {
+            const mars_op_t *op = &m->ops[i];
+            if (op->kind != OP_CONV_I8 || !op->split_next || !op->split_chain) continue;
+            if (!conv_i8_chain_fits(m, op, op + 1, op + 2, op + 3, op->split_chain, n)) {
+                m->no_chain = 1;
                 mars_error_t e = build_plan(m);
                 if (e == MARS_OK) e = upload_params(m);
                 if (e != MARS_OK) return e;
@@ -414,6 +428,8 @@
     if (o->post_next) ADD(" %zd", (ssize_t)o->post_w_off);
     ADD(" split_next %d", o->split_next);
     if (o->split_next) ADD(" %zd", (ssize_t)o->split_w_off);
+    ADD(" split_chain %d", o->split_chain);
+    if (o->split_chain) ADD(" %zd", (ssize_t)o->chain_w_off);
     ADD(" pre %d", o->pre);
     if (o->pre) ADD(" %zd %zd %zd %a", (ssize_t)o->pre_w_off, (ssize_t)o->pre_b_off, (ssize_t)o->pre_lut2_off, (double)o->pre_cs);
     ADD(" macs %a bytes %a prof_kind %d", o->macs, o->bytes, o->prof_kind);
@@ -464,10 +480,10 @@
     if (full) {
         const plan_switches_t *w = &m->sw;
         snprintf(line, sizeof line, "+plan n_ops %d arena_size %zu scratch_per_frame %zu blob_mirror_bytes %zu rec_max_frames %zu rec_skipped %d f32_mode %d | fusion %d"
-                 " no_fuse_lut %d no_nhwc_internal %d no_vconcat_q %d no_pair_f32 %d no_rec %d no_zero_tail %d no_vconcat_f32 %d no_rowpad %d no_post %d no_split %d rec_limit %zu"
+                 " no_fuse_lut %d no_nhwc_internal %d no_vconcat_q %d no_pair_f32 %d no_rec %d no_zero_tail %d no_vconcat_f32 %d no_rowpad %d no_post %d no_split %d no_chain %d rec_limit %zu"
                  " vconcat_limit %zu bottleneck_limit %zu\n", m->n_ops, m->arena_size, m->scratch_per_frame, m->blob_mirror_bytes, m->rec_max_frames, m->rec_skipped,
                  m->plan_f32_mode, w->fusion, w->no_fuse_lut, w->no_nhwc_internal, w->no_vconcat_q, w->no_pair_f32, w->no_rec, w->no_zero_tail, w->no_vconcat_f32,
-                 w->no_rowpad, w->no_post, w->no_split, w->rec_limit, w->vconcat_limit, w->bottleneck_limit);
+                 w->no_rowpad, w->no_post, w->no_split, w->no_chain, w->rec_limit, w->vconcat_limit, w->bottleneck_limit);
         EMIT();
     }
 #undef EMIT
diff --git a/thingino-accel_amd/csrc/host/mars_plan.c b/thingino-accel_amd/csrc/host/mars_plan.c
--- a/thingino-accel_amd/csrc/host/mars_plan.c
+++ b/thingino-accel_amd/csrc/host/mars_plan.c
@@ -640,6 +640,19 @@
     p.lut = p.lut2 = p.split_lut2[0] = p.split_lut2[1] = (const uint8_t *)a;
     p.split_w = (const int8_t *)a; p.split_out[0] = p.split_out[1] = (int8_t *)m;
     p.split_out_stride[0] = planned_stride(&m->mt[b->t_out]); p.split_out_stride[1] = planned_stride(&m->mt[c->t_out]);
+    return mhip_conv_i8_split_ok(&p);
+}
+
+int conv_i8_chain_fits(const mars_model_ext_t *m, const mars_op_t *a, const mars_op_t *b, const mars_op_t *c, const mars_op_t *d, int side, int frames) {
+    mhip_conv_i8_t p;
+    if (a->t_in[0] < 0 || a->t_out < 0 || b->t_out < 0 || c->t_out < 0 || d->t_out < 0 || (side != 1 && side != 2)) return 0;
+    conv_i8_geometry(a, frames, &p);
+    p.in_stride = planned_stride(&m->mt[a->t_in[0]]); p.out_stride = planned_stride(&m->mt[a->t_out]);
+    p.lut = p.lut2 = p.split_lut2[0] = p.split_lut2[1] = p.chain_lut2 = (const uint8_t *)a;
+    p.split_w = p.chain_w = (const int8_t *)a;
+    p.split_out[0] = (int8_t *)m; p.split_out[1] = (int8_t *)m + 1; p.chain_out = (int8_t *)m + 2;
+    p.split_out_stride[0] = planned_stride(&m->mt[b->t_out]); p.split_out_stride[1] = planned_stride(&m->mt[c->t_out]);
+    p.chain_side = side; p.chain_out_stride = planned_stride(&m->mt[d->t_out]);
     return mhip_conv_i8_split_ok(&p);
 }
 
@@ -1155,6 +1168,50 @@
     free(readers);
 }
 
+static int chain_mate_ok(const mars_op_t *d, const mars_op_t *a) {
+    return d->kind == OP_CONV_I8 && d->kh == 1 && d->kw == 1 && d->sh == 1 && d->sw == 1 && !d->pt && !d->pl && d->safe && !d->nchw && !d->out_nchw && !d->add_t &&
+           !d->chain_n && !d->store_c && !d->in_byte_off && !d->out_byte_off && !d->out_pix_stride && !d->out_ch_off && d->lut_off != NO_OFF &&
+           d->lut2_off != NO_OFF && !d->nseg && !d->pre && !d->pair_next && !d->post_next && !d->split_next && d->n_in == 1 && d->in_c == 32 && d->out_c == 32 &&
+           d->oc_pad == 32 && d->row_pad == 32 && d->in_h == a->out_h && d->in_w == a->out_w && d->out_h == a->out_h && d->out_w == a->out_w;
+}
+void fuse_split_chain(mars_model_ext_t *m) {
+    if (m->sw.no_chain || m->no_chain || m->sw.no_split || m->no_split) return;
+    int *readers, *writers;
+    if (!use_counts(m, &readers, &writers)) return;
+    for (int i = 0; i + 3 < m->n_ops; i++) {
+        mars_op_t *a = &m->ops[i];
+        if (a->kind != OP_CONV_I8 || !a->split_next || a->split_chain) continue;
+        const int O0 = a[1].t_out, O1 = a[2].t_out;
+        for (int j = i + 3; j < m->n_ops && j <= i + 48; j++) {
+            const mars_op_t *d = &m->ops[j];
+            if (!chain_mate_ok(d, a) || m->ops[j - 1].pair_next || m->ops[j - 1].post_next || m->ops[j - 1].split_next ||
+                (j >= 2 && m->ops[j - 2].split_next))
+                continue;
+            const int side = d->t_in[0] == O0 ? 1 : (d->t_in[0] == O1 ? 2 : 0), O = d->t_out;
+            if (!side || O < 0 || O == O0 || O == O1 || O == a->t_out || writers[O] != 1 || m->mt[O].io_in || m->mt[O].is_weight || m->mt[O].pix_stride ||
+                op_reads(a, O) || op_reads(d, O))
+                continue;
+            if (touched_between(m, i + 3, j, O, USE_READ | USE_WRITE) || touched_between(m, i + 3, j, d->t_in[0], USE_WRITE)) continue;
+            if (!conv_i8_chain_fits(m, a, a + 1, a + 2, d, side, 1)) continue;
+            const size_t bytes = mhip_conv_i8_chain_pack(NULL, NULL, NULL);
+            const size_t off = arena_reserve(m, bytes);
+            if (off == NO_OFF) { free(readers); return; }
+            mhip_conv_i8_chain_pack((const int8_t *)(m->arena_host + d->w_off), d->b_off != NO_OFF ? (const int32_t *)(m->arena_host + d->b_off) : NULL,
+                                    (int8_t *)(m->arena_host + off));
+            if (j > i + 3) {
+                const mars_op_t moved = *d;
+                memmove(&m->ops[i + 4], &m->ops[i + 3], sizeof(mars_op_t) * (size_t)(j - i - 3));
+                m->ops[i + 3] = moved;
+            }
+            a->split_chain = side;
+            a->chain_w_off = off;
+            break;
+        }
+        i += 2;
+    }
+    free(readers);
+}
+
 void pad_output_rows(mars_model_ext_t *m) {
     for (uint32_t i = 0; i < m->pub.header.num_tensors; i++) m->mt[i].pix_c = m->mt[i].pix_stride = 0;
     if (m->sw.no_rowpad) return;
@@ -1630,6 +1687,11 @@
                                    !m->ops[i + 1].pair_next || m->ops[i + 2].pair_next || m->ops[i + 1].n_in != 1 || m->ops[i + 2].n_in != 1 ||
                                    m->ops[i + 1].t_in[0] != o->t_out || m->ops[i + 2].t_in[0] != o->t_out || o->post_next || o->pair_next || o->pre || o->add_t))
             why = "split_next without its pair of 1x1s behind it";
+        else if (o->split_chain && (!o->split_next || i + 3 >= m->n_ops || !chain_mate_ok(&m->ops[i + 3], o) || (o->split_chain != 1 && o->split_chain != 2) ||
+                                    m->ops[i + 3].t_in[0] != m->ops[i + o->split_chain].t_out || m->ops[i + 3].t_out < 0 ||
+                                    m->ops[i + 3].t_out == m->ops[i + 1].t_out || m->ops[i + 3].t_out == m->ops[i + 2].t_out || m->ops[i + 3].t_out == o->t_out ||
+                                    m->mt[m->ops[i + 3].t_out].pix_stride || o->chain_w_off == NO_OFF))
+            why = "split_chain without its 1x1 behind the pair";
         for (int k = 0; !why && k < o->nseg; k++)
             if (!op_reads(o, o->seg_t[k])) why = "a seg_t is not among t_in";
         for (int k = 0; !why && k < o->vc_n; k++)
diff --git a/thingino-accel_amd/csrc/host/mars_run.c b/thingino-accel_amd/csrc/host/mars_run.c
--- a/thingino-accel_amd/csrc/host/mars_run.c
+++ b/thingino-accel_amd/csrc/host/mars_run.c
@@ -81,6 +81,15 @@
         p->split_cs[k] = side[k]->cs;
         p->split_out[k] = (int8_t *)tdev(m, side[k]->t_out); p->split_out_stride[k] = tstride(m, side[k]->t_out);
     }
+}
+
+static void conv_i8_chain_params(const mars_model_ext_t *m, const mars_op_t *op, const mars_op_t *d, mhip_conv_i8_t *p) {
+    uint8_t *A = m->arena_dev;
+    p->chain_side = op->split_chain;
+    p->chain_w = (const int8_t *)(A + op->chain_w_off);
+    p->chain_lut2 = A + d->lut2_off;
+    p->chain_cs = d->cs;
+    p->chain_out = (int8_t *)tdev(m, d->t_out); p->chain_out_stride = tstride(m, d->t_out);
 }
 
 static void conv_f32_params(mars_model_ext_t *m, mars_op_t *op, mhip_conv_f32_t *p) {
@@ -329,9 +338,11 @@
         }
         mars_op_t *mate = (op->pair_next || op->post_next || op->split_next) && i + 1 < m->n_ops ? &m->ops[i + 1] : NULL;
         mars_op_t *mate2 = op->split_next && i + 2 < m->n_ops ? &m->ops[i + 2] : NULL;
+        mars_op_t *mate3 = op->split_next && op->split_chain && i + 3 < m->n_ops ? &m->ops[i + 3] : NULL;
         if (wait_tail && ((op->t_out >= 0 && (m->mt[op->t_out].io_out || m->mt[op->t_out].tail_read)) ||
                           (mate && mate->t_out >= 0 && (m->mt[mate->t_out].io_out || m->mt[mate->t_out].tail_read)) ||
-                          (mate2 && mate2->t_out >= 0 && (m->mt[mate2->t_out].io_out || m->mt[mate2->t_out].tail_read)))) {
+                          (mate2 && mate2->t_out >= 0 && (m->mt[mate2->t_out].io_out || m->mt[mate2->t_out].tail_read)) ||
+                          (mate3 && mate3->t_out >= 0 && (m->mt[mate3->t_out].io_out || m->mt[mate3->t_out].tail_read)))) {
             mhip_stream_wait(sid, m->ev_tail_done);
             wait_tail = 0;
         }
@@ -348,11 +359,12 @@
         if (op->split_next) {
             mhip_conv_i8_t pa;
             rc = -1;
-            if (mate && mate2) {
+            if (mate && mate2 && (mate3 || !op->split_chain)) {
                 conv_i8_split_params(m, op, mate, mate2, &pa);
+                if (mate3) conv_i8_chain_params(m, op, mate3, &pa);
                 rc = mhip_conv_i8(&pa);
             }
-            i += 2;
+            i += mate3 ? 3 : 2;
         } else if (mate && op->post_next) {
             mhip_conv_i8_t pa;
             conv_i8_post_params(m, op, mate, &pa);
@@ -382,8 +394,8 @@
             rc = launch_op(m, op);
         }
         {
-            const mars_op_t *w2[3] = {op, mate, mate2};
-            for (int q = 0; q < 3; q++)
+            const mars_op_t *w2[4] = {op, mate, mate2, mate3};
+            for (int q = 0; q < 4; q++)
                 if (w2[q] && op_writes(w2[q], m->scratch_t)) m->scratch_t = -1;
         }
         if (m->profiling) {
@@ -725,6 +737,7 @@
         if (op->pair_next || (i > 0 && m->ops[i - 1].pair_next)) continue;
         if (op->post_next || (i > 0 && m->ops[i - 1].post_next)) continue;
         if (op->split_next) continue;
+        if (i >= 3 && m->ops[i - 3].split_chain) continue;
         mhip_conv_i8_t p;
         conv_i8_params(m, op, &p);
         int codes[32];
diff --git a/thingino-accel_amd/csrc/mhip.h b/thingino-accel_amd/csrc/mhip.h
--- a/thingino-accel_amd/csrc/mhip.h
+++ b/thingino-accel_amd/csrc/mhip.h
@@ -83,10 +83,17 @@
     const uint8_t *split_lut2[2];
     float split_cs[2];
     int8_t *split_out[2];   size_t split_out_stride[2];
+    int chain_side;
+    const int8_t *chain_w;
+    const uint8_t *chain_lut2;
+    float chain_cs;
+    int8_t *chain_out;      size_t chain_out_stride;
 } mhip_conv_i8_t;
 int mhip_conv_i8_split_ok(const mhip_conv_i8_t *p);
 size_t mhip_conv_i8_split_pack(const int8_t *packed0, const int32_t *bias0, const int8_t *packed1, const int32_t *bias1, int8_t *out);
 int mhip_conv_i8_split_row(int side, int oc);
+size_t mhip_conv_i8_chain_pack(const int8_t *packed, const int32_t *bias, int8_t *out);
+int mhip_conv_i8_chain_k(int c);
 int mhip_conv_i8_post_ok(const mhip_conv_i8_t *p);
 size_t mhip_conv_i8_post_pack(int c, const int8_t *packed, const int32_t *bias, int8_t *out);
 int mhip_conv_i8_post_k(int c, int k);
```

After: 61440, median of 6. 1.6% higher.
